# malaire/reed-solomon-16

Hardware: AMD Instinct MI355X
Metric: encode+decode GiB/s (device-resident, 1024B shards); % of HBM roofline (higher is better)
Workload: dtype u16; 1 GPU; 32768:32768 x 1024 B encode + 100%-loss decode per GPU (BASELINE configs[3]); original_count=32768, recovery_count=32768, parallelism=independent stripes x 1 (weak, no collective), column_slices=1, decode_issue=serial: rs16_decode_device after the encode

## Files before the change

include/rs16.h:

```cpp
#ifndef RS16_H
#define RS16_H

#include <stddef.h>
#include <stdint.h>

#ifdef __cplusplus
extern "C" {
#endif

typedef enum rs16_error_code {
    RS16_OK = 0,
    RS16_DIFFERENT_SHARD_SIZE = 1,
    RS16_DUPLICATE_ORIGINAL_SHARD_INDEX = 2,
    RS16_DUPLICATE_RECOVERY_SHARD_INDEX = 3,
    RS16_INVALID_ORIGINAL_SHARD_INDEX = 4,
    RS16_INVALID_RECOVERY_SHARD_INDEX = 5,
    RS16_INVALID_SHARD_SIZE = 6,
    RS16_NOT_ENOUGH_SHARDS = 7,
    RS16_TOO_FEW_ORIGINAL_SHARDS = 8,
    RS16_TOO_MANY_ORIGINAL_SHARDS = 9,
    RS16_UNSUPPORTED_SHARD_COUNT = 10,
    RS16_DEVICE_ERROR = 100,
    RS16_INVALID_ARGUMENT = 101
} rs16_error_code;
// ... 108 lines not shown
                        size_t original_received_count, size_t recovery_received_count, void* stream,
                        rs16_error* err);
int rs16_decode_device_prepared(rs16_engine* eng, size_t original_count, size_t recovery_count,
                                size_t shard_bytes, void* d_original, const void* d_recovery, void* stream,
                                rs16_error* err);

enum { RS16_UPDATE_MAX_SHARDS = 32 };
typedef struct rs16_update_plan rs16_update_plan;
rs16_update_plan* rs16_update_plan_new(rs16_engine* eng, int rate, size_t original_count, size_t recovery_count,
                                       const size_t* indices, size_t n, rs16_error* err);
void rs16_update_plan_free(rs16_update_plan* plan);
size_t rs16_update_plan_count(const rs16_update_plan* plan);
int rs16_update_plan_coefficients(rs16_update_plan* plan, uint16_t* out, rs16_error* err);
int rs16_update_device(rs16_update_plan* plan, size_t shard_bytes, const void* d_delta, void* d_recovery,
                       size_t recovery_pos, size_t recovery_n, void* stream, rs16_error* err);

int rs16_encode_host_batch(rs16_engine* eng, size_t original_count, size_t recovery_count, size_t shard_bytes,
                           size_t nstripes, const void* h_original, size_t original_stride, void* h_recovery,
                           size_t recovery_stride, rs16_error* err);
int rs16_decode_host_batch(rs16_engine* eng, size_t original_count, size_t recovery_count, size_t shard_bytes,
                           size_t nstripes, void* h_original, size_t original_stride,
                           const uint8_t* original_received, size_t original_received_stride,
                           const void* h_recovery, size_t recovery_stride, const uint8_t* recovery_received,
                           size_t recovery_received_stride, rs16_error* err);

int rs16_encode_host_multi(rs16_engine* const* engines, int n, size_t original_count, size_t recovery_count,
                           size_t shard_bytes, const void* h_original, void* h_recovery, rs16_error* err);
int rs16_decode_host_multi(rs16_engine* const* engines, int n, size_t original_count, size_t recovery_count,
                           size_t shard_bytes, void* h_original, const uint8_t* original_received,
                           const void* h_recovery, const uint8_t* recovery_received, rs16_error* err);

typedef struct rs16_comm rs16_comm;
int rs16_comm_unique_id(void* id128, rs16_error* err);
rs16_comm* rs16_comm_new(rs16_engine* eng, int nranks, int rank, const void* id128, rs16_error* err);
int rs16_comm_init_all(rs16_engine* const* engines, int n, rs16_comm** comms, rs16_error* err);
void rs16_comm_free(rs16_comm* comm);
int rs16_comm_rank(const rs16_comm* comm);
int rs16_comm_size(const rs16_comm* comm);
int rs16_column_slice(size_t shard_bytes, int nranks, int rank, size_t* offset, size_t* width);
int rs16_scatter_columns(rs16_comm* const* comms, int n, int root, size_t rows, size_t shard_bytes,
                         const void* const* d_full, void* const* d_slice, void* stream, rs16_error* err);
int rs16_gather_columns(rs16_comm* const* comms, int n, int root, size_t rows, size_t shard_bytes,
                        const void* const* d_slice, void* const* d_full, void* stream, rs16_error* err);
int rs16_scatter_columns_virtual(rs16_comm* comm, int vslices, size_t rows, size_t shard_bytes, const void* d_full,
                                 void* const* d_slices, void* stream, rs16_error* err);
int rs16_gather_columns_virtual(rs16_comm* comm, int vslices, size_t rows, size_t shard_bytes,
                                const void* const* d_slices, void* d_full, void* stream, rs16_error* err);

void* rs16_device_alloc(rs16_engine* eng, size_t bytes, rs16_error* err);
void rs16_device_free(rs16_engine* eng, void* d_ptr);
int rs16_memcpy_htod(rs16_engine* eng, void* d_dst, const void* src, size_t bytes, void* stream, rs16_error* err);
int rs16_memcpy_dtoh(rs16_engine* eng, void* dst, const void* d_src, size_t bytes, void* stream, rs16_error* err);
int rs16_memset_device(rs16_engine* eng, void* d_dst, int value, size_t bytes, void* stream, rs16_error* err);
int rs16_memcpy2d_htod(rs16_engine* eng, void* d_dst, size_t d_pitch, const void* src, size_t h_pitch, size_t width,
                       size_t rows, void* stream, rs16_error* err);
int rs16_memcpy2d_dtoh(rs16_engine* eng, void* dst, size_t h_pitch, const void* d_src, size_t d_pitch, size_t width,
                       size_t rows, void* stream, rs16_error* err);
void* rs16_stream_create(rs16_engine* eng, rs16_error* err);
void rs16_stream_destroy(rs16_engine* eng, void* stream);
void* rs16_host_alloc(rs16_engine* eng, size_t bytes, rs16_error* err);
void rs16_host_free(rs16_engine* eng, void* h_ptr);

int rs16_engine_set_profiling(rs16_engine* eng, int enable, rs16_error* err);
int rs16_engine_profile_read(rs16_engine* eng, int prog, double* total_ms, uint64_t* launches, rs16_error* err);
void rs16_engine_profile_reset(rs16_engine* eng);
int rs16_prog_count(void);
int rs16_engine_set_stamps(rs16_engine* eng, void* d_buf, int prog, rs16_error* err);
const char* rs16_prog_name(int prog);

enum {
    RS16_DIAG_FORCE_VOFF64 = 1,
    RS16_DIAG_EVAL_TWO_KERNEL = 2,
    RS16_DIAG_EVAL_FULL = 4,
    RS16_DIAG_NO_COLUMN = 8,
    RS16_DIAG_FORCE_COLUMN = 16,
    RS16_DIAG_TILE_LAST = 32,
    RS16_DIAG_NO_TILE_LAST = 64,
    RS16_DIAG_FD_LDS = 128,
    RS16_DIAG_COL_RADIX4 = 256,
    RS16_DIAG_NO_IDENTITY = 512,
    RS16_DIAG_NO_MID_DIRECT = 1024,
    RS16_DIAG_WIDE_TWIDDLES = 2048,
    RS16_DIAG_NO_LATE_ROWS = 4096,
    RS16_DIAG_NO_PAIRED_ROWS = 8192
};
int rs16_engine_set_diagnostics(rs16_engine* eng, int flags);
int rs16_set_diagnostics(int flags);

void rs16_host_mul(const void* in, void* out, size_t bytes, uint16_t log_m);
void rs16_host_mul_narrow(const void* in, void* out, size_t bytes, uint16_t log_m);
uint32_t rs16_host_twiddle(uint32_t index, uint32_t* log_m, uint32_t* table20);
int rs16_host_twiddle_narrow(uint32_t index);
uint64_t rs16_host_fast_div_check(uint32_t divisor, uint32_t n0, uint32_t count, uint32_t step);
typedef struct rs16_pass_consts {
    uint32_t voff32, full_lanes, nslab;
    uint32_t quads, threads, load_shb, store_shb, reg_bits, row_sets;
    uint64_t rs_in, rs_seg, rs_out;
    uint32_t late_rows;
} rs16_pass_consts;
int rs16_host_pass_consts(int prog, int T, uint32_t lo, uint64_t s_in, uint64_t s_out, uint64_t s_seg, uint64_t s_rest,
                          uint32_t qrow, uint32_t chunk, uint32_t row_base_in, uint32_t in_rows_mask, int diag,
                          rs16_pass_consts* out);
int rs16_host_pass_consts_many(int prog, int T, uint32_t lo, size_t n, const uint64_t* s_in, const uint64_t* s_out,
                               const uint64_t* s_seg, const uint64_t* s_rest, const uint32_t* qrow, uint32_t chunk,
                               uint32_t row_base_in, uint32_t in_rows_mask, int diag, rs16_pass_consts* out);
int rs16_host_pass_consts_rows(int prog, int T, uint32_t lo, uint64_t s_in, uint64_t s_out, uint64_t s_seg,
                               uint64_t s_rest, uint32_t qrow, uint32_t chunk, uint32_t row_base_in,
                               uint32_t in_rows_mask, uint32_t a_count, int diag, rs16_pass_consts* out);
int rs16_host_paired_rows(uint32_t chunk_rows, uint64_t S, uint64_t S_user, uint32_t a_count, uint32_t seg_chunk,
                          uint32_t row_base_in, int diag);
int rs16_host_update_consts(uint32_t rows, uint64_t shard_bytes, uint32_t n, uint32_t* quads_per_lane,
                            uint32_t* nslab, uint32_t* rows_per_wave, uint64_t* blocks);

const char* rs16_version(void);

#ifdef __cplusplus
}
#endif
#endif
```

reed-solomon-16_amd/csrc/rs16_api.cpp:

```cpp
#include <atomic>
#include <rccl/rccl.h>

#include <cstdio>

#include "rs16_api.hpp"
#include "rs16_pass_common.hpp"

using namespace rs16;

extern "C" size_t rs16_error_message(const rs16_error* e, char* buf, size_t len) {
    char tmp[256];
    unsigned long long a = e->v0, b = e->v1, c = e->v2;
    switch (e->code) {
    case RS16_OK: snprintf(tmp, sizeof tmp, "ok"); break;
    case RS16_DIFFERENT_SHARD_SIZE:
        snprintf(tmp, sizeof tmp, "different shard size: expected %llu bytes, got %llu bytes", a, b);
        break;
    case RS16_DUPLICATE_ORIGINAL_SHARD_INDEX: snprintf(tmp, sizeof tmp, "duplicate original shard index: %llu", a); break;
    case RS16_DUPLICATE_RECOVERY_SHARD_INDEX: snprintf(tmp, sizeof tmp, "duplicate recovery shard index: %llu", a); break;
    case RS16_INVALID_ORIGINAL_SHARD_INDEX:
        snprintf(tmp, sizeof tmp, "invalid original shard index: %llu >= original_count %llu", b, a);
        break;
    case RS16_INVALID_RECOVERY_SHARD_INDEX:
        snprintf(tmp, sizeof tmp, "invalid recovery shard index: %llu >= recovery_count %llu", b, a);
        break;
    case RS16_INVALID_SHARD_SIZE:
        snprintf(tmp, sizeof tmp, "invalid shard size: %llu bytes (must non-zero and multiple of 64)", a);
        break;
    case RS16_NOT_ENOUGH_SHARDS:
        snprintf(tmp, sizeof tmp, "not enough shards: %llu original + %llu recovery < %llu original_count", b, c, a);
        break;
    case RS16_TOO_FEW_ORIGINAL_SHARDS:
        snprintf(tmp, sizeof tmp, "too few original shards: got %llu shards while original_count is %llu", b, a);
        break;
    case RS16_TOO_MANY_ORIGINAL_SHARDS:
        snprintf(tmp, sizeof tmp, "too many original shards: got more than original_count (%llu) shards", a);
        break;
    case RS16_UNSUPPORTED_SHARD_COUNT:
        snprintf(tmp, sizeof tmp, "unsupported shard count: %llu original shards with %llu recovery shards", a, b);
        break;
    case RS16_DEVICE_ERROR:
        if (a >= 1000)
            snprintf(tmp, sizeof tmp, "device error: RCCL: %s", ncclGetErrorString((ncclResult_t)(a - 1000)));
        else
            snprintf(tmp, sizeof tmp, "device error: %s", hipGetErrorString((hipError_t)a));
        break;
    case RS16_INVALID_ARGUMENT: snprintf(tmp, sizeof tmp, "invalid argument"); break;
    default: snprintf(tmp, sizeof tmp, "unknown error %d", e->code); break;
    }
    size_t n = strlen(tmp);
    if (buf && len) {
        size_t c2 = std::min(n, len - 1);
        memcpy(buf, tmp, c2);
        buf[c2] = 0;
    }
    return n;
}

template <class Mul> static void host_mul(const void* in, void* out, size_t bytes, uint16_t log_m, Mul mul) {
    const uint32_t* t = &host_tables().mul_tab[(size_t)log_m * TAB_DWORDS];
    const uint8_t* src = (const uint8_t*)in;
    uint8_t* dst = (uint8_t*)out;
    for (size_t q = 0; q < bytes / 8; q++) {
        const size_t off = (q >> 3) * 64 + (q & 7) * 4;
        uint32_t yl, yh, ol = 0, oh = 0;
        memcpy(&yl, src + off, 4);
        memcpy(&yh, src + off + 32, 4);
        mul(ol, oh, yl, yh, t);
        memcpy(dst + off, &ol, 4);
        memcpy(dst + off + 32, &oh, 4);
    }
}
extern "C" void rs16_host_mul(const void* in, void* out, size_t bytes, uint16_t log_m) {
    host_mul(in, out, bytes, log_m, mul_xor);
}
extern "C" void rs16_host_mul_narrow(const void* in, void* out, size_t bytes, uint16_t log_m) {
    host_mul(in, out, bytes, log_m, mul_xor_narrow);
}
extern "C" uint32_t rs16_host_twiddle(uint32_t index, uint32_t* log_m, uint32_t* table20) {
    const HostTables& t = host_tables();
    if (index >= GF_MODULUS) return ~0u;
    if (log_m) *log_m = t.skew[index];
    if (table20) memcpy(table20, &t.skew_tab[(size_t)index * TAB_DWORDS], 20 * sizeof(uint32_t));
    return t.skew[index] == GF_MODULUS ? 0u : t.exp[t.skew[index]];
}
extern "C" int rs16_host_twiddle_narrow(uint32_t index) { return twiddle_narrow(index) ? 1 : 0; }
extern "C" uint64_t rs16_host_fast_div_check(uint32_t divisor, uint32_t n0, uint32_t count, uint32_t step) {
    const FastDiv f = fast_div_of(divisor);
    uint64_t bad = 0;
    for (uint64_t i = 0, n = n0; i < count && n < ((uint64_t)1 << 32); i++, n += step)
        bad += fast_div((uint32_t)n, f.mul, f.one) != (uint32_t)n / divisor;
    return bad;
}

static int host_pass_consts(int prog, int T, uint32_t lo, size_t n, const uint64_t* s_in, const uint64_t* s_out,
                            const uint64_t* s_seg, const uint64_t* s_rest, const uint32_t* qrow, uint32_t chunk,
                            uint32_t row_base_in, uint32_t in_rows_mask, uint32_t a_count, int diag,
                            rs16_pass_consts* out) {
    if (prog < 0 || prog >= NUM_PROGS || T < 0 || T > 8 || !out) return 0;
    const PassKernel& k = pass_kernel_of(prog, T);
    if (!k.fn) return 0;
    PassArgs a{};
    a.lo = lo, a.chunk = chunk, a.row_base_in = row_base_in, a.in_rows_mask = in_rows_mask;
    a.diag = (uint32_t)diag;
    a.a_count = a_count;
    for (size_t i = 0; i < n; i++) {
        a.S_in = s_in[i], a.S_out = s_out[i], a.S_seg = s_seg[i], a.S_rest = s_rest[i], a.qrow = qrow[i];
        const PassConsts c = pass_launch_consts(k, T, a);
        rs16_pass_consts& o = out[i];
        o.voff32 = c.voff32, o.full_lanes = c.full_lanes, o.nslab = c.nslab;
        o.quads = (uint32_t)k.quads, o.threads = (uint32_t)k.threads;
        o.load_shb = (uint32_t)k.load_shb, o.store_shb = (uint32_t)k.store_shb;
        o.reg_bits = (uint32_t)k.reg_bits, o.row_sets = k.quads >= 64 ? 1u : 64u / (uint32_t)k.quads;
        o.rs_in = c.rs_in, o.rs_seg = c.rs_seg, o.rs_out = c.rs_out;
        o.late_rows = c.late_rows;
    }
    return 1;
}
extern "C" int rs16_host_pass_consts_many(int prog, int T, uint32_t lo, size_t n, const uint64_t* s_in,
                                          const uint64_t* s_out, const uint64_t* s_seg, const uint64_t* s_rest,
                                          const uint32_t* qrow, uint32_t chunk, uint32_t row_base_in,
                                          uint32_t in_rows_mask, int diag, rs16_pass_consts* out) {
    return host_pass_consts(prog, T, lo, n, s_in, s_out, s_seg, s_rest, qrow, chunk, row_base_in, in_rows_mask, 0, diag,
                            out);
}
extern "C" int rs16_host_pass_consts_rows(int prog, int T, uint32_t lo, uint64_t s_in, uint64_t s_out, uint64_t s_seg,
                                          uint64_t s_rest, uint32_t qrow, uint32_t chunk, uint32_t row_base_in,
                                          uint32_t in_rows_mask, uint32_t a_count, int diag, rs16_pass_consts* out) {
    return host_pass_consts(prog, T, lo, 1, &s_in, &s_out, &s_seg, &s_rest, &qrow, chunk, row_base_in, in_rows_mask,
                            a_count, diag, out);
}
extern "C" int rs16_host_pass_consts(int prog, int T, uint32_t lo, uint64_t s_in, uint64_t s_out, uint64_t s_seg,
                                     uint64_t s_rest, uint32_t qrow, uint32_t chunk, uint32_t row_base_in,
                                     uint32_t in_rows_mask, int diag, rs16_pass_consts* out) {
    return rs16_host_pass_consts_many(prog, T, lo, 1, &s_in, &s_out, &s_seg, &s_rest, &qrow, chunk, row_base_in,
                                      in_rows_mask, diag, out);
}
extern "C" int rs16_host_paired_rows(uint32_t chunk_rows, uint64_t S, uint64_t S_user, uint32_t a_count,
                                     uint32_t seg_chunk, uint32_t row_base_in, int diag) {
    return paired_rows_sequence(chunk_rows, S, S_user, a_count, seg_chunk, row_base_in, diag) ? 1 : 0;
}
extern "C" int rs16_host_update_consts(uint32_t rows, uint64_t shard_bytes, uint32_t n, uint32_t* quads_per_lane,
                                       uint32_t* nslab, uint32_t* rows_per_wave, uint64_t* blocks) {
    if (shard_bytes == 0 || (shard_bytes & 63) != 0 || shard_bytes / 8 > 0xFFFFFFFFu) return 0;
    UpdateArgs a{};
    a.S = shard_bytes, a.qrow = (uint32_t)(shard_bytes / 8), a.rows = rows;
    uint64_t nb;
    if (!update_launch_consts(a, n, &nb)) return 0;
    if (quads_per_lane) *quads_per_lane = a.quads_per_lane;
    if (nslab) *nslab = a.nslab;
    if (rows_per_wave) *rows_per_wave = a.rows_per_wave;
    if (blocks) *blocks = nb;
    return 1;
}

extern "C" int rs16_engine_set_profiling(rs16_engine* e, int enable, rs16_error* err) {
    if (int rc = e->activate(err)) return rc;
    if (int rc = e->prof_collect(err)) return rc;
    e->profiling = enable != 0;
    return set_error(err, RS16_OK);
}
extern "C" int rs16_engine_profile_read(rs16_engine* e, int prog, double* total_ms, uint64_t* launches,
                                        rs16_error* err) {
    if (prog < 0 || prog >= NUM_PROF) return set_error(err, RS16_INVALID_ARGUMENT);
    if (int rc = e->activate(err)) return rc;
    if (int rc = e->prof_collect(err)) return rc;
    if (total_ms) *total_ms = e->prof_ms[prog];
    if (launches) *launches = e->prof_n[prog];
    return set_error(err, RS16_OK);
}
extern "C" void rs16_engine_profile_reset(rs16_engine* e) {
    rs16_error err;
    (void)e->activate(&err);
    (void)e->prof_collect(&err);
    for (int i = 0; i < NUM_PROF; i++) e->prof_ms[i] = 0, e->prof_n[i] = 0;
}
extern "C" int rs16_engine_set_stamps(rs16_engine* e, void* d_buf, int prog, rs16_error* err) {
    if (prog < -1 || prog >= NUM_PROF) return set_error(err, RS16_INVALID_ARGUMENT);
    e->stamp_buf = d_buf;
    e->stamp_prof = prog;
    return set_error(err, RS16_OK);
}
extern "C" int rs16_engine_set_slices(rs16_engine* e, int n, rs16_error* err) {
    if (n < 1 || n > rs16_engine::MAX_SLICES) return set_error(err, RS16_INVALID_ARGUMENT);
    e->slices = n;
    return set_error(err, RS16_OK);
}
extern "C" int rs16_decode_check(rs16_engine* e, void* stream, rs16_error* err) {
    if (!e->last_dec_valid && !e->last_dec_flags_only) return set_error(err, RS16_OK);
    if (int rc = e->activate(err)) return rc;
    RS16_HIP(hipStreamSynchronize(e->pick(stream)));
    const DecodeGeom& g = e->last_dec;
    uint64_t a = 0, b = 0;
    if (e->last_dec_flags_only) {
        std::vector<uint8_t> f(2 * (size_t)GF_ORDER);
        RS16_HIP(hipMemcpy(f.data(), e->ws_flags.p, f.size(), hipMemcpyDeviceToHost));
        for (uint32_t i = 0; i < g.a_count; i++) a += f[i] != 0;
        for (uint32_t i = 0; i < g.b_count; i++) b += f[GF_ORDER + i] != 0;
    } else {
        const size_t chunks = ((size_t)g.n + 63) / 64;
        std::vector<uint32_t> c(2 * chunks);
        RS16_HIP(hipMemcpy(c.data(), e->ev_main.rcount.p, c.size() * 4, hipMemcpyDeviceToHost));
        for (size_t i = 0; i < chunks; i++) a += c[2 * i], b += c[2 * i + 1];
    }
    const auto want = DecodeSides::by_segment<uint64_t>(g.high, g.a_recv, g.b_recv);
    const auto got = DecodeSides::by_segment<uint64_t>(g.high, a, b);
    if (got != want) return set_error(err, RS16_INVALID_ARGUMENT, got.first, got.second);
    return set_error(err, RS16_OK);
}
static constexpr int DIAG_ALL = DIAG_FORCE_VOFF64 | DIAG_EVAL_TWO_KERNEL | DIAG_EVAL_FULL | DIAG_NO_COLUMN |
                                DIAG_FORCE_COLUMN | DIAG_TILE_LAST | DIAG_NO_TILE_LAST | DIAG_FD_LDS |
                                DIAG_COL_RADIX4 | DIAG_NO_IDENTITY | DIAG_NO_MID_DIRECT | DIAG_WIDE_TWIDDLES |
                                DIAG_NO_LATE_ROWS | DIAG_NO_PAIRED_ROWS;
extern "C" int rs16_engine_set_diagnostics(rs16_engine* e, int flags) {
    const int old = e->diag;
    e->diag = flags & DIAG_ALL;
    return old;
}
static std::atomic<int> g_default_diag{0};
extern "C" int rs16_set_diagnostics(int flags) { return g_default_diag.exchange(flags & DIAG_ALL); }
extern "C" int rs16_prog_count(void) { return NUM_PROF; }
extern "C" const char* rs16_prog_name(int prog) {
    static const char* names[] = {"GEN_FFT",   "GEN_IFFT",   "ENC_FIRST",     "ENC_MID",
                                  "ENC_LAST",  "ENC_SINGLE", "DEC_FIRST",     "DEC_MID",
                                  "DEC_LAST",  "DEC_SINGLE", "DEC_HALF_LAST", "DEC_HALF_SINGLE",
                                  "DEC_HALF_FIRST", "DEC_HALF_MID", "EVAL_POLY", "COL_ENC", "COL_DEC",
                                  "DEC_MID_DIRECT", "DEC_TILE_LAST"};
    static_assert(sizeof names / sizeof names[0] == NUM_PROF, "profiling names");
    return (prog >= 0 && prog < NUM_PROF) ? names[prog] : "?";
}

extern "C" const char* rs16_version(void) { return "rs16-mi355x 0.1 gfx950 (v_perm GF(2^16) engine)"; }

static bool high_supports(size_t k, size_t m) {
    return k > 0 && m > 0 && k < GF_ORDER && m < GF_ORDER && next_pow2(m) + k <= GF_ORDER;
}
static bool low_supports(size_t k, size_t m) {
    return k > 0 && m > 0 && k < GF_ORDER && m < GF_ORDER && next_pow2(k) + m <= GF_ORDER;
}

extern "C" int rs16_use_high_rate(size_t k, size_t m, rs16_error* err) {
    if (k > GF_ORDER || m > GF_ORDER) return set_error(err, RS16_UNSUPPORTED_SHARD_COUNT, k, m), -1;
    const size_t kp = next_pow2(k), mp = next_pow2(m);
    const size_t smaller = std::min(kp, mp), larger = std::max(k, m);
    if (k == 0 || m == 0 || smaller + larger > GF_ORDER) return set_error(err, RS16_UNSUPPORTED_SHARD_COUNT, k, m), -1;
    set_error(err, RS16_OK);
    if (kp < mp) return 0;
    if (kp > mp) return 1;
    return k <= m ? 1 : 0;
}

extern "C" int rs16_supports(int rate, size_t k, size_t m) {
    if (rate == RS16_RATE_HIGH) return high_supports(k, m);
    if (rate == RS16_RATE_LOW) return low_supports(k, m);
    return rs16_use_high_rate(k, m, nullptr) >= 0;
}

extern "C" int rs16_validate(int rate, size_t k, size_t m, size_t S, rs16_error* err) {
    if (!rs16_supports(rate, k, m)) return set_error(err, RS16_UNSUPPORTED_SHARD_COUNT, k, m);
    if (S == 0 || (S & 63) != 0 || (uint64_t)S >> 32) return set_error(err, RS16_INVALID_SHARD_SIZE, S);
    return set_error(err, RS16_OK);
}

extern "C" size_t rs16_encoder_work_count(int high, size_t k, size_t m) {
    const size_t chunk = high ? next_pow2(m) : next_pow2(k);
    const size_t n = high ? k : m;
    return (n + chunk - 1) / chunk * chunk;
}
extern "C" size_t rs16_decoder_work_count(int high, size_t k, size_t m) {
    return decode_geom(high != 0, k, m).n;
}

int rs16::resolve_rate(int rate, size_t k, size_t m, size_t S, bool* high, rs16_error* err) {
    if (rate == RS16_RATE_DEFAULT) {
        int h = rs16_use_high_rate(k, m, err);
        if (h < 0) return err ? err->code : RS16_UNSUPPORTED_SHARD_COUNT;
        *high = h == 1;
    } else if (rate == RS16_RATE_HIGH || rate == RS16_RATE_LOW) {
        *high = rate == RS16_RATE_HIGH;
    } else {
        return set_error(err, RS16_INVALID_ARGUMENT);
    }
    return rs16_validate(*high ? RS16_RATE_HIGH : RS16_RATE_LOW, k, m, S, err);
}
int rs16::check_received(size_t k, size_t orig_recv, size_t rec_recv, rs16_error* err) {
    if (orig_recv + rec_recv < k) return set_error(err, RS16_NOT_ENOUGH_SHARDS, k, orig_recv, rec_recv);
    return RS16_OK;
}

extern "C" rs16_engine* rs16_engine_new(int device, rs16_error* err) { return rs16_engine_new_ex(device, 0, err); }

extern "C" rs16_engine* rs16_engine_new_ex(int device, int flags, rs16_error* err) {
    if (flags & ~RS16_ENGINE_OWN_QUEUE) return set_error(err, RS16_INVALID_ARGUMENT), nullptr;
    int ndev = 0;
    hipError_t he = hipGetDeviceCount(&ndev);
    if (he != hipSuccess) return hip_fail(err, he), nullptr;
    if (device < 0 || device >= ndev) return set_error(err, RS16_INVALID_ARGUMENT), nullptr;
    rs16_engine* e = new (std::nothrow) rs16_engine();
    if (!e) return set_error(err, RS16_INVALID_ARGUMENT), nullptr;
    e->device = device;
    e->diag = g_default_diag.load();
    const HostTables& t = host_tables();
    auto fail = [&](hipError_t x) {
        hip_fail(err, x);
        rs16_engine_free(e);
        return (rs16_engine*)nullptr;
    };
    if ((he = hipSetDevice(device)) != hipSuccess) return fail(he);
    if (flags & RS16_ENGINE_OWN_QUEUE) {
        int cus = 0;
        if ((he = hipDeviceGetAttribute(&cus, hipDeviceAttributeMultiprocessorCount, device)) != hipSuccess) return fail(he);
        std::vector<uint32_t> mask(((size_t)cus + 31) / 32, 0xFFFFFFFFu);
        if (cus % 32) mask.back() = (1u << (cus % 32)) - 1;
        if ((he = hipExtStreamCreateWithCUMask(&e->stream, (uint32_t)mask.size(), mask.data())) != hipSuccess)
            return fail(he);
    } else if ((he = hipStreamCreateWithFlags(&e->stream, hipStreamNonBlocking)) != hipSuccess) {
        return fail(he);
    }
    e->flags = flags;
    if ((he = hipMalloc(&e->d_skew_tab, (size_t)GF_ORDER * TAB_DWORDS * 4)) != hipSuccess) return fail(he);
    if ((he = hipMalloc(&e->d_mul_tab, t.mul_tab.size() * 4)) != hipSuccess) return fail(he);
    if ((he = hipMalloc(&e->d_log_walsh, GF_ORDER * 2)) != hipSuccess) return fail(he);
    if ((he = hipMalloc(&e->d_zero_sink, RS16_ZERO_BYTES)) != hipSuccess) return fail(he);
    if ((he = hipMemset(e->d_zero_sink, 0, RS16_ZERO_BYTES)) != hipSuccess) return fail(he);
    if ((he = hipMemcpy(e->d_skew_tab, t.skew_tab.data(), t.skew_tab.size() * 4, hipMemcpyHostToDevice)) != hipSuccess) return fail(he);
    if ((he = hipMemcpy(e->d_mul_tab, t.mul_tab.data(), t.mul_tab.size() * 4, hipMemcpyHostToDevice)) != hipSuccess) return fail(he);
    if ((he = hipMemcpy(e->d_log_walsh, t.log_walsh.data(), GF_ORDER * 2, hipMemcpyHostToDevice)) != hipSuccess) return fail(he);
    set_error(err, RS16_OK);
    return e;
}

extern "C" void rs16_engine_free(rs16_engine* e) {
    if (!e) return;
    (void)hipSetDevice(e->device);
    if (e->stream) (void)hipStreamSynchronize(e->stream);
    for (int j = 0; j < rs16_engine::MAX_SLICES; j++)
        if (e->sl_own[j]) (void)hipStreamSynchronize(e->sl_own[j]);
    for (auto& sl : e->hslot)
        if (sl.s) (void)hipStreamSynchronize(sl.s);
    if (e->last == rs16_engine::LAST_CALLER && e->order_ev) (void)hipEventSynchronize(e->order_ev);
    for (rs16_encoder* c : e->encoders) detach(c);
    for (rs16_decoder* c : e->decoders) detach(c);
    for (rs16_update_plan* c : e->update_plans) detach(c);
    e->ws_z.release();
    e->ws_u.release();
    e->ws_fd.release();
    for (auto& b : e->mid_tab) b.release();
    e->ev_main.release();
    for (auto& l : e->ev_lane) l.release();
    e->ws_flags.release();
    e->hp_flags.release();
    for (auto& sl : e->hslot) {
        if (sl.s) (void)hipStreamSynchronize(sl.s), (void)hipStreamDestroy(sl.s);
        sl.orig.release(), sl.rec.release(), sl.z.release(), sl.u.release();
    }
    e->hflags.release();
    if (e->hev) (void)hipEventDestroy(e->hev);
    if (e->prep_ev) (void)hipEventDestroy(e->prep_ev);
    for (auto& ev : e->hp_ev)
        if (ev) (void)hipEventDestroy(ev);
    if (e->hp_off) (void)hipEventDestroy(e->hp_off);
    if (e->order_ev) (void)hipEventDestroy(e->order_ev);
    for (int j = 0; j < rs16_engine::MAX_SLICES; j++) {
        if (e->sl_own[j]) (void)hipStreamDestroy(e->sl_own[j]);
        if (e->sl_join[j]) (void)hipEventDestroy(e->sl_join[j]);
    }
    if (e->sl_fork) (void)hipEventDestroy(e->sl_fork);
    if (e->d_skew_tab) (void)hipFree(e->d_skew_tab);
    if (e->d_mul_tab) (void)hipFree(e->d_mul_tab);
    if (e->d_col_img) (void)hipFree(e->d_col_img);
    if (e->d_col_v) (void)hipFree(e->d_col_v);
    if (e->d_log_walsh) (void)hipFree(e->d_log_walsh);
    if (e->d_zero_sink) (void)hipFree(e->d_zero_sink);
    if (e->stream) (void)hipStreamDestroy(e->stream);
    delete e;
}

extern "C" int rs16_engine_device(const rs16_engine* e) { return e->device; }
extern "C" void* rs16_engine_stream(const rs16_engine* e) { return (void*)e->stream; }
extern "C" int rs16_engine_synchronize(rs16_engine* e, void* stream, rs16_error* err) {
    if (int rc = e->activate(err)) return rc;
    RS16_HIP(hipStreamSynchronize(e->pick(stream)));
    return set_error(err, RS16_OK);
}

static bool is_pow2(size_t x) { return x && !(x & (x - 1)); }

static int check_transform(size_t shard_count, size_t S, size_t pos, size_t size, size_t trunc, size_t skew_delta,
                           rs16_error* err) {
    if (S == 0 || (S & 63) || !is_pow2(size) || size > GF_ORDER || trunc > size || pos + size > shard_count)
        return set_error(err, RS16_INVALID_ARGUMENT);
    if (size >= 2 && size - 2 + skew_delta >= GF_MODULUS) return set_error(err, RS16_INVALID_ARGUMENT);
    return RS16_OK;
}

extern "C" int rs16_engine_fft(rs16_engine* e, void* data, size_t shard_count, size_t S, size_t pos, size_t size,
                               size_t trunc, size_t skew_delta, void* stream, rs16_error* err) {
    if (int rc = check_transform(shard_count, S, pos, size, trunc, skew_delta, err)) return rc;
    if (!shard_aligned(data)) return set_error(err, RS16_INVALID_ARGUMENT);
    if (int rc = e->activate(err)) return rc;
    if (int rc = e->fft((uint8_t*)data, S, pos, size, skew_delta, e->pick(stream), err)) return rc;
    return set_error(err, RS16_OK);
}
extern "C" int rs16_engine_fft_skew_end(rs16_engine* e, void* data, size_t shard_count, size_t S, size_t pos,
                                        size_t size, size_t trunc, void* stream, rs16_error* err) {
    return rs16_engine_fft(e, data, shard_count, S, pos, size, trunc, pos + size, stream, err);
}
extern "C" int rs16_engine_ifft(rs16_engine* e, void* data, size_t shard_count, size_t S, size_t pos, size_t size,
                                size_t trunc, size_t skew_delta, void* stream, rs16_error* err) {
    if (int rc = check_transform(shard_count, S, pos, size, trunc, skew_delta, err)) return rc;
    if (!shard_aligned(data)) return set_error(err, RS16_INVALID_ARGUMENT);
    if (int rc = e->activate(err)) return rc;
    if (int rc = e->ifft((uint8_t*)data, S, pos, size, skew_delta, e->pick(stream), err)) return rc;
    return set_error(err, RS16_OK);
}
extern "C" int rs16_engine_ifft_skew_end(rs16_engine* e, void* data, size_t shard_count, size_t S, size_t pos,
                                         size_t size, size_t trunc, void* stream, rs16_error* err) {
    return rs16_engine_ifft(e, data, shard_count, S, pos, size, trunc, pos + size, stream, err);
}
extern "C" int rs16_engine_fwht(rs16_engine* e, uint16_t* d, size_t trunc, void* stream, rs16_error* err) {
    if (trunc > GF_ORDER) return set_error(err, RS16_INVALID_ARGUMENT);
    if (int rc = e->activate(err)) return rc;
    if (int rc = e->order(e->pick(stream), err)) return rc;
    if (int rc = e->guard_eval(e->pick(stream), false, err)) return rc;
    RS16_HIP(e->evset->work32.reserve(GF_ORDER * 4));
    RS16_HIP(launch_fwht_u16(d, (uint32_t*)e->evset->work32.p, e->pick(stream)));
    if (int rc = e->scratch_done(e->pick(stream), err)) return rc;
    return set_error(err, RS16_OK);
}
extern "C" int rs16_engine_eval_poly(rs16_engine* e, uint16_t* d, size_t trunc, void* stream, rs16_error* err) {
    if (trunc > GF_ORDER) return set_error(err, RS16_INVALID_ARGUMENT);
    if (int rc = e->activate(err)) return rc;
    if (int rc = e->order(e->pick(stream), err)) return rc;
    if (int rc = e->guard_eval(e->pick(stream), false, err)) return rc;
    RS16_HIP(e->evset->work32.reserve(GF_ORDER * 4));
    RS16_HIP(launch_eval_poly_u16(d, (uint32_t*)e->evset->work32.p, e->d_log_walsh, e->pick(stream)));
    if (int rc = e->scratch_done(e->pick(stream), err)) return rc;
    return set_error(err, RS16_OK);
}
extern "C" int rs16_engine_mul(rs16_engine* e, void* x, size_t bytes, uint16_t log_m, void* stream, rs16_error* err) {
    if ((bytes & 63) || !shard_aligned(x)) return set_error(err, RS16_INVALID_ARGUMENT);
    if (int rc = e->activate(err)) return rc;
    RS16_HIP(launch_mul((uint8_t*)x, bytes, log_m, e->d_mul_tab, e->pick(stream)));
    return set_error(err, RS16_OK);
}
extern "C" int rs16_engine_xor(rs16_engine* e, void* x, const void* y, size_t bytes, void* stream, rs16_error* err) {
    if ((bytes & 63) || !shard_aligned(x) || !shard_aligned(y)) return set_error(err, RS16_INVALID_ARGUMENT);
    if (int rc = e->activate(err)) return rc;
    RS16_HIP(launch_xor((uint8_t*)x, (const uint8_t*)y, bytes, e->pick(stream)));
    return set_error(err, RS16_OK);
}
// ... 88 lines not shown
```

reed-solomon-16_amd/csrc/rs16_engine.cpp:

```cpp
#include <cstdlib>
#include "rs16_engine.hpp"

#include <algorithm>
#include <cstring>

namespace rs16 {

hipError_t DevBuf::reserve(size_t bytes) {
    if (bytes <= cap) return hipSuccess;
    if (p) (void)hipFree(p);
    p = nullptr;
    cap = 0;
    hipError_t e = hipMalloc(&p, bytes);
    if (e == hipSuccess) cap = bytes;
    return e;
}
void DevBuf::release() {
    if (p) (void)hipFree(p);
    p = nullptr;
    cap = 0;
}

hipError_t HostBuf::reserve(size_t bytes) {
    if (bytes <= cap) return hipSuccess;
// ... 265 lines not shown
}

int rs16_engine::fft(uint8_t* data, size_t S, size_t pos, size_t size, size_t skew_delta, hipStream_t s,
                     rs16_error* err) {
    const int L = ilog2(size);
    if (L == 0) return RS16_OK;
    PassArgs a = base_args(this, S);
    a.in = a.out = data + pos * S;
    a.skew_fft = (uint32_t)skew_delta;
    if (L <= 8) {
        RS16_PASS(GEN_FFT, L, a, 1, s);
        return RS16_OK;
    }
    const int lo = L / 2, hi = L - lo;
    a.lo = lo;
    RS16_PASS(GEN_FFT, hi, a, 1u << lo, s);
    a.lo = 0;
    RS16_PASS(GEN_FFT, lo, a, 1u << hi, s);
    return RS16_OK;
}

int rs16_engine::ifft(uint8_t* data, size_t S, size_t pos, size_t size, size_t skew_delta, hipStream_t s,
                      rs16_error* err) {
    const int L = ilog2(size);
    if (L == 0) return RS16_OK;
    PassArgs a = base_args(this, S);
    a.in = a.out = data + pos * S;
    a.skew_ifft = (uint32_t)skew_delta;
    if (L <= 8) {
        RS16_PASS(GEN_IFFT, L, a, 1, s);
        return RS16_OK;
    }
    const int lo = L / 2, hi = L - lo;
    a.lo = 0;
    RS16_PASS(GEN_IFFT, lo, a, 1u << hi, s);
    a.lo = lo;
    RS16_PASS(GEN_IFFT, hi, a, 1u << lo, s);
    return RS16_OK;
}

int rs16_engine::encode_high_fused(size_t k, size_t m, size_t S, size_t S_user, const uint8_t* d_orig, uint8_t* d_rec, uint8_t* Z,
                                   hipStream_t s, rs16_error* err, size_t nst, size_t bs_orig, size_t bs_rec) {
    const size_t chunk = next_pow2(m);
    const int L = ilog2(chunk);
    PassArgs a = base_args(this, S);
    a.seg_a = d_orig;
    a.S_seg = S_user;
    a.a_count = (uint32_t)k;
    a.skew_ifft = (uint32_t)chunk;
    a.skew_fft = 0;
    a.out_rows = (uint32_t)m;
    const uint32_t ns = (uint32_t)nst;
    auto batch = [&](uint32_t tiles, size_t bs_in, size_t bs_out, size_t bs_seg) {
        a.stripe_tiles = ns > 1 ? tiles : 0;
        a.bs_in = bs_in;
        a.bs_out = bs_out;
        a.bs_seg = bs_seg;
        return tiles * ns;
    };
    if (col_ok(L, S, nst)) {
        ColArgs c = col_args();
        c.in = d_orig;
        c.out = d_rec;
        c.S_in = c.S_out = S_user;
        c.qrow = (uint32_t)(S / 8);
        c.nstripes = ns;
        c.bs_in = bs_orig;
        c.bs_out = bs_rec;
        c.in_rows = (uint32_t)k;
        c.out_rows = (uint32_t)m;
        c.skew_ifft = (uint32_t)chunk;
        c.skew_fft = 0;
        return col(c, L, COL_ENC, s, err);
    }
    if (L <= 8) {
        a.out = d_rec;
        a.S_out = S_user;
        RS16_PASS(ENC_SINGLE, L, a, batch(1, 0, bs_rec, bs_orig), s);
        return RS16_OK;
    }
    const int lo = L / 2, hi = L - lo;
    const size_t zs = chunk * S;
    const bool paired = paired_rows_sequence((uint32_t)chunk, S, S_user, a.a_count, a.chunk, a.row_base_in, diag);
    a.out = Z;
    a.lo = 0;
    a.paired = paired ? paired_sides_of(ENC_FIRST) : 0;
    RS16_PASS(ENC_FIRST, lo, a, batch(1u << hi, 0, zs, bs_orig), s);
    a.in = Z;
    a.lo = lo;
    a.paired = paired ? paired_sides_of(ENC_MID) : 0;
    RS16_PASS(ENC_MID, hi, a, batch(1u << lo, zs, zs, 0), s);
    a.in = Z;
    a.out = d_rec;
    a.S_out = S_user;
    a.lo = 0;
    a.paired = paired ? paired_sides_of(ENC_LAST) : 0;
    const uint32_t tiles = (uint32_t)((m + ((size_t)1 << lo) - 1) >> lo);
    RS16_PASS(ENC_LAST, lo, a, batch(tiles, zs, bs_rec, 0), s);
    return RS16_OK;
}

int rs16_engine::decode_fused(const DecodeGeom& g, size_t S, size_t S_user, const uint8_t* seg_a, const uint8_t* flags_a,
                              const uint8_t* seg_b, const uint8_t* flags_b, uint8_t* rest, uint8_t* Z, uint8_t* U,
                              hipStream_t s, rs16_error* err) {
    if (int rc = decode_eval(g, flags_a, flags_b, s, err, S)) return rc;
    return decode_passes(g, S, S_user, seg_a, flags_a, seg_b, flags_b, rest, Z, U, (uint32_t*)evset->rcount.p, s, err);
}

int rs16_engine::guard_eval(hipStream_t s, bool consume, rs16_error* err) {
    if (!prep_pending) return RS16_OK;
    RS16_HIP(hipStreamWaitEvent(s, prep_ev, 0));
    prep_pending = false;
    if (!consume) prep.valid = false;
    return RS16_OK;
}

int rs16_engine::decode_eval(const DecodeGeom& g, const uint8_t* flags_a, const uint8_t* flags_b, hipStream_t s,
                             rs16_error* err, size_t S, size_t nstripes, uint32_t vary, size_t bs_fa, size_t bs_fb) {
    if (evset == &ev_main && !preparing)
        if (int rc = guard_eval(s, false, err)) return rc;
    if (!preparing) prep.valid = false;
    const size_t nv = vary > 1 ? vary : 1;
    RS16_HIP(evset->work32.reserve(nv * VARY_WORK * 4));
    RS16_HIP(evset->elog.reserve(nv * VARY_WORK * 4));
    RS16_HIP(evset->zflag.reserve(nv * VARY_ZFLAGS));
    RS16_HIP(evset->rbits.reserve(nv * VARY_RBITS * 4));
    RS16_HIP(evset->lost.reserve(nv * VARY_LOST * 4));
    RS16_HIP(evset->rcount.reserve(GF_ORDER / 64 * 8));
    var_ns = vary > 1 ? vary : 0;
    var_bs_fa = vary > 1 ? bs_fa : 0;
    var_bs_fb = vary > 1 ? bs_fb : 0;
    ErasureSpec es{};
    es.flags_a = flags_a;
    es.flags_b = flags_b;
    es.a_count = g.a_count;
    es.chunk = g.chunk;
    es.b_count = g.b_count;
    es.pad_fill = g.high ? 1 : 0;
    es.tail_fill = g.high ? 0 : 1;
    const int L = ilog2(g.n);
    es.rbits = (uint32_t*)evset->rbits.p;
    es.zflags = L > 8 ? (uint8_t*)evset->zflag.p : nullptr;
    es.n = g.n;
    es.zlo = (uint32_t)(L / 2);
    const bool prune = !half_decode(g) && L > 8;
    es.lostpart = prune ? (uint32_t*)evset->lost.p : nullptr;
    es.lostrange = prune ? (uint32_t*)evset->lost.p + 512 : nullptr;
    es.orig_b = g.high ? 1 : 0;
    es.rcount = (uint32_t*)evset->rcount.p;
    es.diag = (uint32_t)diag;
    last_dec = g;
    last_dec_valid = true;
    if (var_ns) {
        es.nstripes = var_ns;
        es.bs_fa = var_bs_fa;
        es.bs_fb = var_bs_fb;
        es.bs_work = es.bs_elog = VARY_WORK;
        es.bs_rbits = VARY_RBITS;
        es.bs_zflags = VARY_ZFLAGS;
        es.bs_lost = VARY_LOST;
        es.rcount = nullptr;
        last_dec_valid = false;
    }
    e_ident = identity_logs(g, vary);
    if (e_ident) {
        eval_in_col = elog_fused = false;
        return RS16_OK;
    }
    eval_in_col = S && (half_decode(g) ? g.high && col_ok(ilog2(g.n) - 1, S, nstripes)
                                       : col_ok(ilog2(g.n), S, nstripes, true));
    if (eval_in_col) return RS16_OK;
    es.stamps = stamp_prof == PROF_EVAL_POLY ? (uint64_t*)stamp_buf : nullptr;
    hipEvent_t pev;
    if (int rc = prof_begin(s, &pev, err)) return rc;
    const bool small = g.high && g.n <= 2048 && !(diag & DIAG_EVAL_FULL);
    elog_fused = !(half_decode(g) && ilog2(g.n) - 1 <= 8);
    if (small) {
        RS16_HIP(launch_eval_poly_small(es, (uint32_t)g.n, (uint32_t*)evset->work32.p, (uint32_t*)evset->elog.p, d_log_walsh,
                                        s, !elog_fused));
// ... 11 lines not shown

bool rs16_engine::identity_logs(const DecodeGeom& g, uint32_t vary) const {
    if ((diag & DIAG_NO_IDENTITY) || vary > 1 || !half_decode(g) || ilog2(g.n) - 1 < 11) return false;
    if (g.a_count != g.chunk || g.b_count != g.chunk) return false;
    return g.high ? g.a_recv == g.a_count : g.b_recv == g.b_count;
}

int rs16_engine::mid_tables(int L, const uint32_t** out, rs16_error* err) {
    DevBuf& b = mid_tab[L];
    if (!b.p) {
        const HostTables& t = host_tables();
        const std::vector<uint32_t> ent = mid_matrix_entries(t, L);
        std::vector<uint32_t> tabs(ent.size() * 20);
        for (size_t i = 0; i < ent.size(); i++)
            std::copy_n(&t.mul_tab[(size_t)ent[i] * TAB_DWORDS], 20, &tabs[i * 20]);
        hipError_t he = b.reserve(tabs.size() * 4);
        if (he == hipSuccess) he = hipMemcpy(b.p, tabs.data(), tabs.size() * 4, hipMemcpyHostToDevice);
        if (he != hipSuccess) {
            b.release();
            return hip_fail(err, he);
        }
    }
    *out = (const uint32_t*)b.p;
    return RS16_OK;
}

int rs16_engine::decode_passes(const DecodeGeom& g, size_t S, size_t S_user, const uint8_t* seg_a, const uint8_t* flags_a,
                               const uint8_t* seg_b, const uint8_t* flags_b, uint8_t* rest, uint8_t* Z, uint8_t* U,
                               uint32_t* rcount, hipStream_t s, rs16_error* err, size_t nst, size_t bs_a, size_t bs_b,
                               size_t bs_rest) {
    PassArgs a = base_args(this, S);
    a.S_seg = a.S_rest = S_user;
    a.seg_a = seg_a;
    a.seg_b = seg_b;
    a.flags_a = flags_a;
    a.flags_b = flags_b;
    a.a_count = g.a_count;
    a.chunk = g.chunk;
    a.b_count = g.b_count;
    a.elog = (const uint32_t*)evset->elog.p;
    a.ework = elog_fused ? (const uint32_t*)evset->work32.p : nullptr;
    a.rest = rest;
    a.rest_seg_b = g.high ? 1 : 0;
    a.rbits = (const uint32_t*)evset->rbits.p;
    a.skew_ifft = a.skew_fft = 0;
    if (var_ns) {
        a.bs_fa = var_bs_fa;
        a.bs_fb = var_bs_fb;
        a.bs_elog = VARY_WORK;
        a.bs_rbits = VARY_RBITS;
        a.bs_zflags = VARY_ZFLAGS;
        a.bs_lost = VARY_LOST;
        rcount = nullptr;
    }
    const uint32_t ns = (uint32_t)nst;
    const size_t zs = (size_t)g.n * S;
    a.bs_seg = bs_a;
    a.bs_seg_b = bs_b;
    a.bs_rest = bs_rest;
    auto batch = [&](uint32_t tiles, size_t bs_in, size_t bs_in2, size_t bs_out) {
        a.stripe_tiles = ns > 1 ? tiles : 0;
        a.bs_in = bs_in;
        a.bs_in2 = bs_in2;
        a.bs_out = bs_out;
        return tiles * ns;
    };
    const int L = ilog2(g.n);
    if (half_decode(g)) {
        const uint32_t half = g.n / 2, src = g.high ? 0 : half, dst = g.high ? half : 0;
        const uint32_t orig = g.high ? g.b_count : g.a_count;
        a.row_base_in = a.skew_ifft = src;
        a.row_base_out = a.skew_fft = dst;
        const int Lh = L - 1;
        if (e_ident) {
            const int lo = Lh / 2, hi = Lh - lo;
            a.seg_a = g.high ? seg_a : seg_b;
            a.bs_seg = g.high ? bs_a : bs_b;
            a.a_count = half;
            a.rcount = rcount;
            a.cnt_flags = g.high ? flags_a : flags_b;
            a.cnt_base = src;
            a.cnt_seg = g.high ? 0 : 1;
            const bool paired = paired_rows_sequence(half, S, S_user, a.a_count, a.chunk, a.row_base_in, diag);
            a.lo = 0;
            a.out = Z;
            a.paired = paired ? paired_sides_of(ENC_FIRST) : 0;
            RS16_PASS_AS(PROF_DEC_HALF_FIRST, ENC_FIRST, lo, a, batch(1u << hi, 0, 0, zs), s);
            a.rcount = nullptr;
            a.lo = lo;
            a.in = Z;
            a.paired = paired ? paired_sides_of(ENC_MID) : 0;
            RS16_PASS_AS(PROF_DEC_HALF_MID, ENC_MID, hi, a, batch(1u << lo, zs, 0, zs), s);
            a.lo = 0;
            a.out = rest;
            a.S_out = S_user;
            a.out_rows = orig;
            a.paired = paired ? paired_sides_of(ENC_LAST) : 0;
            a.rcount = rcount;
            a.cnt_flags = g.high ? flags_b : flags_a;
            a.cnt_base = dst;
            a.cnt_seg = g.high ? 1 : 0;
            RS16_PASS_AS(DEC_HALF_LAST, ENC_LAST, lo, a, batch((orig + (1u << lo) - 1) >> lo, zs, 0, bs_rest), s);
            return RS16_OK;
        }
        const bool col_eval = eval_in_col && g.high;
        if (!col_eval && Lh <= 8) {
            a.ework = nullptr;
            RS16_PASS(DEC_HALF_SINGLE, Lh, a, batch(1, 0, 0, 0), s);
            return RS16_OK;
        }
        if (col_eval || col_ok(Lh, S, ns)) {
            ColArgs c = col_args();
            c.in = g.high ? seg_a : seg_b;
            c.flags = g.high ? flags_a : flags_b;
            c.in_rows = g.high ? g.a_count : g.b_count;
            c.out = rest;
            c.S_in = c.S_out = S_user;
            c.qrow = (uint32_t)(S / 8);
            c.nstripes = ns;
            c.bs_in = g.high ? bs_a : bs_b;
            c.bs_out = bs_rest;
            c.out_rows = orig;
            c.base_in = c.skew_ifft = src;
            c.base_out = c.skew_fft = dst;
            c.chunk = g.chunk;
            c.e_pad = 1;
            c.bs_flags = g.high ? var_bs_fa : var_bs_fb;
            c.bs_flags_o = var_bs_fb;
            c.bs_elog = var_ns ? VARY_WORK : 0;
            if (col_eval) {
                c.flags_o = flags_b;
                c.o_rows = g.b_count;
                c.vtab = nullptr;
                c.rcount = rcount;
                return col(c, Lh, COL_DEC_EVAL, s, err);
            }
            c.elog = (const uint32_t*)evset->work32.p;
            return col(c, Lh, COL_DEC_EWORK, s, err);
        }
        const int lo = Lh / 2, hi = Lh - lo;
        a.paired = 0;
        a.lo = 0;
        a.out = Z;
        RS16_PASS_AS(PROF_DEC_HALF_FIRST, DEC_FIRST, lo, a, batch(1u << hi, 0, 0, zs), s);
        a.lo = lo;
        a.in = Z;
        RS16_PASS_AS(PROF_DEC_HALF_MID, ENC_MID, hi, a, batch(1u << lo, zs, 0, zs), s);
        a.lo = 0;
        a.out = nullptr;
        RS16_PASS(DEC_HALF_LAST, lo, a, batch((orig + (1u << lo) - 1) >> lo, zs, 0, 0), s);
        return RS16_OK;
    }
    if (eval_in_col) {
        ColArgs c = col_args();
        c.in = seg_a;
        c.flags = flags_a;
        c.in_rows = g.a_count;
        c.in_b = seg_b;
        c.bs_in_b = bs_b;
        c.flags_o = flags_b;
        c.o_rows = g.b_count;
        c.chunk = g.chunk;
        c.rev_a = g.high ? 0 : 1;
        c.e_pad = g.high ? 1 : 0;
        c.e_tail = g.high ? 0 : 1;
        c.e_k = g.high ? 0 : host_tables().col_k[L];
        c.out = rest;
        c.S_in = c.S_out = S_user;
        c.qrow = (uint32_t)(S / 8);
        c.nstripes = ns;
        c.bs_in = bs_a;
        c.bs_out = bs_rest;
        c.out_rows = g.high ? g.b_count : g.a_count;
        c.rcount = rcount;
        c.bs_flags = var_bs_fa;
        c.bs_flags_o = var_bs_fb;
        return col(c, L, COL_DEC_GEN, s, err);
    }
    if (L <= 8) {
        RS16_PASS(DEC_SINGLE, L, a, batch(1, 0, 0, 0), s);
// ... 206 lines not shown
```

reed-solomon-16_amd/csrc/rs16_engine.hpp:

```cpp
#pragma once
#include <cstddef>
#include <cstdint>
#include <vector>

#include "../../include/rs16.h"
#include "rs16_internal.hpp"

namespace rs16 {

struct DevBuf {
    void* p = nullptr;
    size_t cap = 0;
    hipError_t reserve(size_t bytes);
    void release();
};
struct HostBuf {
    void* p = nullptr;
    size_t cap = 0;
    hipError_t reserve(size_t bytes);
    void release();
};
struct Pending {
    hipEvent_t ev = nullptr;
    bool busy = false;
    hipError_t record(hipStream_t s);
    hipError_t wait();
    void release();
};

int set_error(rs16_error* err, int code, uint64_t v0 = 0, uint64_t v1 = 0, uint64_t v2 = 0);
int hip_fail(rs16_error* err, hipError_t e);
#define RS16_HIP(call)                                 \
    do {                                               \
        hipError_t _e = (call);                        \
        if (_e != hipSuccess) return hip_fail(err, _e); \
    } while (0)
#define RS16_PASS(...)                                       \
    do {                                                     \
        if (int _rc = this->pass(__VA_ARGS__, err)) return _rc; \
    } while (0)
#define RS16_PASS_AS(PROF, ...)                                     \
    do {                                                            \
        if (int _rc = this->pass(__VA_ARGS__, err, PROF)) return _rc; \
    } while (0)

size_t next_pow2(size_t x);
inline int ilog2(size_t x) { int l = 0; while (((size_t)1 << l) < x) l++; return l; }

struct DecodeGeom {
    bool high;
    uint32_t a_count, chunk, b_count, n;
    size_t a_recv = 1, b_recv = 1;
};
DecodeGeom decode_geom(bool high, size_t k, size_t m);

}

struct rs16_encoder;
struct rs16_decoder;
struct rs16_update_plan;

struct rs16_engine {
    int device = 0;
    int flags = 0;
    hipStream_t stream = nullptr;
    int diag = 0;
    uint32_t* d_skew_tab = nullptr;
    uint32_t* d_mul_tab = nullptr;
    uint32_t* d_col_img = nullptr;
    uint32_t* d_col_v = nullptr;
    uint16_t* d_log_walsh = nullptr;
    uint8_t* d_zero_sink = nullptr;
    rs16::DevBuf ws_z, ws_u, ws_fd, ws_flags;
    rs16::DevBuf mid_tab[17];
    struct EvalBufs {
        rs16::DevBuf work32, elog;
        rs16::DevBuf zflag;
        rs16::DevBuf rbits;
        rs16::DevBuf lost;
        rs16::DevBuf rcount;
        void release() { work32.release(), elog.release(), zflag.release(), rbits.release(), lost.release(), rcount.release(); }
    };
    EvalBufs ev_main, ev_lane[2];
    EvalBufs* evset = &ev_main;
    struct Prepared {
        bool valid = false, nothing = false;
        size_t k = 0, m = 0, S = 0;
        rs16::DecodeGeom g{};
        const uint8_t* fl_a = nullptr;
        const uint8_t* fl_b = nullptr;
        int nslices = 1;
    } prep;
    hipEvent_t prep_ev = nullptr;
    bool prep_pending = false;
    bool preparing = false;
    int guard_eval(hipStream_t s, bool consume, rs16_error* err);
    rs16::DecodeGeom last_dec{};
    bool last_dec_valid = false;
    bool last_dec_flags_only = false;
    void forget_decode() { last_dec_valid = last_dec_flags_only = false; }
    struct HostSlot {
        hipStream_t s = nullptr;
        rs16::DevBuf orig, rec, z, u;
        rs16::DevBuf rcount;
    };
    HostSlot hslot[2];
    static constexpr int MAX_SLICES = 4;
    int slices = 1;
    hipStream_t sl_stream[MAX_SLICES] = {};
    hipStream_t sl_own[MAX_SLICES] = {};
    hipEvent_t sl_fork = nullptr, sl_join[MAX_SLICES] = {};
    int slice_count(size_t S) const;
    int fork(hipStream_t s, int n, rs16_error* err);
    int join(hipStream_t s, int n, rs16_error* err);
    rs16::DevBuf hflags;
    hipEvent_t hev = nullptr;
    hipEvent_t hp_ev[2] = {};
    hipEvent_t hp_off = nullptr;
    rs16::HostBuf hp_flags;
    int host_pipe_events(rs16_error* err);
    int host_slots(rs16_error* err);

    hipStream_t pick(void* s) const { return s ? (hipStream_t)s : stream; }
    int activate(rs16_error* err);

    enum { LAST_NONE, LAST_ENGINE, LAST_CALLER } last = LAST_NONE;
    hipEvent_t order_ev = nullptr;
    int order(hipStream_t s, rs16_error* err);
    int scratch_done(hipStream_t s, rs16_error* err);

    std::vector<rs16_encoder*> encoders;
    std::vector<rs16_decoder*> decoders;
    std::vector<rs16_update_plan*> update_plans;

    int pass(int prog, int T, const rs16::PassArgs& a, uint32_t tiles, hipStream_t s, rs16_error* err,
             int prof = -1);
    int prof_begin(hipStream_t s, hipEvent_t* ev, rs16_error* err);
    int prof_end(int id, hipStream_t s, hipEvent_t ev, rs16_error* err);
    template <class F> int profiled(int prof, hipStream_t s, rs16_error* err, F launch);
    bool profiling = false;
    void* stamp_buf = nullptr;
    int stamp_prof = -1;
    bool elog_fused = false;
    bool eval_in_col = false;
    bool e_ident = false;
    struct ProfRec {
        int id;
        hipEvent_t a, b;
    };
    std::vector<ProfRec> prof_pending;
// ... 44 lines not shown
```

reed-solomon-16_amd/csrc/rs16_gf.hpp:

```cpp
#pragma once
#include <stdint.h>

#if defined(__HIPCC__) || defined(__HIP__)
#include <hip/hip_runtime.h>
#define RS16_HD __host__ __device__ __forceinline__
#else
#define RS16_HD inline
#endif

namespace rs16 {

constexpr uint32_t GF_ORDER = 65536;
constexpr uint32_t GF_MODULUS = 65535;
constexpr uint32_t ZERO_ENTRY = 65536;
constexpr uint32_t TAB_ENTRIES = 65537;
constexpr uint32_t TAB_DWORDS = 32;

RS16_HD uint32_t perm_sw(uint32_t hi, uint32_t lo, uint32_t sel) {
    uint64_t pool = ((uint64_t)hi << 32) | lo;
    uint32_t r = 0;
    for (int i = 0; i < 4; i++) {
        uint32_t s = (sel >> (8 * i)) & 0xFF;
        r |= (uint32_t)((pool >> (8 * s)) & 0xFF) << (8 * i);
    }
    return r;
}

#if defined(__HIP_DEVICE_COMPILE__)
__device__ __forceinline__ uint32_t perm(uint32_t hi, uint32_t lo, uint32_t sel) {
    return __builtin_amdgcn_perm(hi, lo, sel);
}
__device__ __forceinline__ uint32_t xor3(uint32_t a, uint32_t b, uint32_t c) {
    return __builtin_amdgcn_bitop3_b32(a, b, c, 0x96);
}
#else
inline uint32_t perm(uint32_t hi, uint32_t lo, uint32_t sel) { return perm_sw(hi, lo, sel); }
inline uint32_t xor3(uint32_t a, uint32_t b, uint32_t c) { return a ^ b ^ c; }
#endif

struct MulSel {
    uint32_t s0, s1, s2, s3, s4, s5;
};
RS16_HD MulSel mul_selectors(uint32_t yL, uint32_t yH) {
#if defined(__HIP_DEVICE_COMPILE__)
    const uint64_t y = ((uint64_t)yH << 32) | yL;
    uint64_t a, b;
    asm("v_lshrrev_b64 %0, 3, %1" : "=v"(a) : "v"(y));
    asm("v_lshrrev_b64 %0, 6, %1" : "=v"(b) : "v"(y));
    const uint32_t s0 = yL & 0x07070707u;
    const uint32_t s1 = (uint32_t)a & 0x07070707u;
    const uint32_t s2 = (uint32_t)b & 0x03030303u;
    const uint32_t s3 = yH & 0x07070707u;
    const uint32_t s4 = (uint32_t)(a >> 32) & 0x07070707u;
    const uint32_t s5 = (uint32_t)(b >> 32) & 0x03030303u;
#else
    const uint32_t s0 = yL & 0x07070707u;
    const uint32_t a = yL >> 3;
    const uint32_t s1 = a & 0x07070707u;
    const uint32_t s2 = (a >> 3) & 0x03030303u;
    const uint32_t s3 = yH & 0x07070707u;
    const uint32_t b = yH >> 3;
    const uint32_t s4 = b & 0x07070707u;
    const uint32_t s5 = (b >> 3) & 0x03030303u;
#endif
    return MulSel{s0, s1, s2, s3, s4, s5};
}
template <bool NARROW>
RS16_HD void mul_xor_sel(uint32_t& xL, uint32_t& xH, const MulSel& y, const uint32_t* t) {
    const uint32_t s0 = y.s0, s1 = y.s1, s2 = y.s2, s3 = y.s3, s4 = y.s4, s5 = y.s5;
    if constexpr (NARROW) {
        const uint32_t l0 = perm(t[1], t[0], s0);
        const uint32_t l1 = perm(t[5], t[4], s1);
        const uint32_t l3 = perm(t[9], t[8], s3), h3 = perm(t[11], t[10], s3);
        const uint32_t l4 = perm(t[13], t[12], s4), h4 = perm(t[15], t[14], s4);
        const uint32_t l2 = perm(t[16], t[16], s2);
        const uint32_t l5 = perm(t[18], t[18], s5), h5 = perm(t[19], t[19], s5);
        xL = xor3(xor3(xL, l0, l1), xor3(l2, l3, l4), l5);
        xH = xor3(xH, h3, h4) ^ h5;
    } else {
        const uint32_t l0 = perm(t[1], t[0], s0), h0 = perm(t[3], t[2], s0);
        const uint32_t l1 = perm(t[5], t[4], s1), h1 = perm(t[7], t[6], s1);
        const uint32_t l3 = perm(t[9], t[8], s3), h3 = perm(t[11], t[10], s3);
        const uint32_t l4 = perm(t[13], t[12], s4), h4 = perm(t[15], t[14], s4);
        const uint32_t l2 = perm(t[16], t[16], s2), h2 = perm(t[17], t[17], s2);
        const uint32_t l5 = perm(t[18], t[18], s5), h5 = perm(t[19], t[19], s5);
        xL = xor3(xor3(xL, l0, l1), xor3(l2, l3, l4), l5);
        xH = xor3(xor3(xH, h0, h1), xor3(h2, h3, h4), h5);
    }
}
template <bool NARROW>
RS16_HD void mul_xor_t(uint32_t& xL, uint32_t& xH, uint32_t yL, uint32_t yH, const uint32_t* t) {
    mul_xor_sel<NARROW>(xL, xH, mul_selectors(yL, yH), t);
}
RS16_HD void mul_xor(uint32_t& xL, uint32_t& xH, uint32_t yL, uint32_t yH, const uint32_t* t) {
    mul_xor_t<false>(xL, xH, yL, yH, t);
}
RS16_HD void mul_xor_narrow(uint32_t& xL, uint32_t& xH, uint32_t yL, uint32_t yH, const uint32_t* t) {
    mul_xor_t<true>(xL, xH, yL, yH, t);
}

RS16_HD uint32_t add_mod(uint32_t x, uint32_t y) {
    uint32_t s = x + y;
    return (s + (s >> 16)) & 0xFFFFu;
}
RS16_HD uint32_t sub_mod(uint32_t x, uint32_t y) {
    uint32_t d = x - y;
    return (d + (d >> 16)) & 0xFFFFu;
}

}
```

reed-solomon-16_amd/csrc/rs16_internal.hpp:

```cpp
#pragma once
#include <hip/hip_runtime.h>
#include <stddef.h>
#include <stdint.h>

#include <vector>

#include "rs16_gf.hpp"

namespace rs16 {

struct HostTables {
    std::vector<uint16_t> exp, log, skew, log_walsh;
    std::vector<uint32_t> skew_entry;
    std::vector<uint32_t> mul_tab;
    std::vector<uint32_t> skew_tab;
    std::vector<uint32_t> col_img;
    std::vector<uint32_t> col_v;
    std::vector<uint32_t> col_k;
};
std::vector<uint32_t> mid_matrix_entries(const HostTables& t, int L);

constexpr uint32_t COL_LMIN = 6, COL_LMAX = 10;
constexpr uint32_t COL_LGEN = 11;
constexpr uint32_t COL_LCHUNK = 8;
constexpr uint32_t col_img_count(uint32_t L) {
    return L == COL_LGEN ? 1u : (L >= COL_LCHUNK ? (1u << (16 - L)) : 2u);
}
constexpr size_t col_img_offset(uint32_t L, uint32_t d) {
    size_t off = 0;
    for (uint32_t l = COL_LMIN; l < L; l++) off += (size_t)col_img_count(l) * ((1u << l) - 1) * 20;
    return off + (size_t)d * ((1u << L) - 1) * 20;
}
constexpr size_t COL_IMG_DWORDS = col_img_offset(COL_LGEN + 1, 0);
constexpr size_t col_v_offset(uint32_t n) { return n - (1u << COL_LMIN); }
constexpr size_t COL_V_DWORDS = col_v_offset(4u << COL_LMAX);
const HostTables& host_tables();

RS16_HD bool twiddle_narrow(uint32_t i) {
    const uint32_t x = i + 1;
    return x < ((x & (0u - x)) << 8);
}
inline int first_narrow_layer(uint32_t lo, int T, uint32_t skew, uint32_t bh_max) {
    int k = T;
    for (int kb = T - 1; kb >= 0; kb--) {
        const uint64_t d = (uint64_t)1 << (lo + kb);
        const uint64_t xmax = (((uint64_t)bh_max + 1) << (lo + T)) - d + skew;
        const uint64_t low = (d + skew) & (2 * d - 1);
        const uint64_t bit = low ? (low & (0 - low)) : 2 * d;
        if (xmax >= (bit << 8)) break;
        k = kb;
    }
    return k;
}

enum Prog : int {
    GEN_FFT = 0,
    GEN_IFFT,
    ENC_FIRST,
    ENC_MID,
    ENC_LAST,
    ENC_SINGLE,
    DEC_FIRST,
    DEC_MID,
    DEC_LAST,
    DEC_SINGLE,
    DEC_HALF_LAST,
    DEC_HALF_SINGLE,
    NUM_PROGS
};
enum ProfId : int {
    PROF_DEC_HALF_FIRST = NUM_PROGS,
    PROF_DEC_HALF_MID,
    PROF_EVAL_POLY,
    PROF_COL_ENC,
    PROF_COL_DEC,
    PROF_DEC_MID_DIRECT,
    PROF_DEC_TILE_LAST,
    NUM_PROF
};

struct PassArgs {
    uint8_t* out;
    const uint8_t* in;
    const uint8_t* in2;
    const uint8_t* seg_a;
    const uint8_t* seg_b;
    const uint8_t* flags_a;
    const uint8_t* flags_b;
    uint8_t* rest;
    const uint32_t* elog;
    const uint32_t* skew_tab;
    const uint32_t* mul_tab;
    uint64_t S_in, S_out, S_seg, S_rest;
    uint32_t qrow;
    uint32_t nslab;
    uint32_t ntiles;
    uint32_t lo;
    uint32_t a_count, chunk, b_count;
// ... 16 lines not shown
    uint32_t in_rows_mask;
    uint64_t bs_fa, bs_fb;
    uint32_t bs_elog, bs_rbits, bs_zflags, bs_lost;
    uint32_t diag;
    uint32_t* rcount;
    const uint8_t* cnt_flags;
    uint32_t cnt_base, cnt_seg;
    uint32_t mid_direct;
    uint32_t tl_max;
    uint64_t rs_in, rs_seg, rs_out;
    uint32_t full_lanes;
    uint32_t nslab_one, stripe_one;
    uint32_t paired;
    uint64_t nslab_mul, stripe_mul;
};

struct FastDiv {
    uint64_t mul;
    uint32_t one;
};
inline FastDiv fast_div_of(uint32_t d) {
    if (d <= 1) return {0, ~0u};
    return {~(uint64_t)0 / d + 1, 0};
}
RS16_HD uint32_t fast_div(uint32_t n, uint64_t mul, uint32_t one) {
    const uint64_t lo = ((uint64_t)n * (uint32_t)mul) >> 32;
    return (uint32_t)(((uint64_t)n * (uint32_t)(mul >> 32) + lo) >> 32) + (n & one);
}

struct ColArgs {
    const uint8_t* img_ifft;
    const uint8_t* img_fft;
    const uint8_t* flags_o;
    uint32_t o_rows;
    const uint32_t* vtab;
    uint32_t* rcount;
    uint32_t chunk;
    uint32_t e_pad, e_tail, e_k;
    uint32_t rev_a;
    const uint8_t* in_b;
    uint64_t bs_in_b;
    const uint8_t* in;
    const uint8_t* flags;
    uint8_t* out;
    const uint32_t* elog;
    const uint32_t* skew_tab;
    const uint32_t* mul_tab;
    const uint8_t* zero;
    uint64_t S_in, S_out;
    uint32_t qrow;
    uint32_t nstripes;
    uint32_t in_rows, out_rows;
    uint32_t skew_ifft, skew_fft;
    uint32_t base_in, base_out;
    uint64_t bs_in, bs_out;
    uint64_t bs_flags, bs_flags_o;
    uint32_t bs_elog;
    uint32_t nch;
    uint64_t* stamps;
    uint32_t diag;
};
int col_rows_ok(uint32_t L);
enum ColMode : int { COL_ENC = 0, COL_DEC_EWORK, COL_DEC_EVAL, COL_DEC_GEN, COL_ENC_IFFT, COL_ENC_FFTX };
constexpr uint32_t COL_MAX_CHUNKS = 64;
hipError_t launch_col(const ColArgs& a, uint32_t L, int mode, hipStream_t s);
constexpr uint32_t COLM_L = 7, COLM_MAX_CHUNKS = 16;
hipError_t launch_col_multi(const ColArgs& a, bool high, hipStream_t s);

enum DiagFlags : int {
    DIAG_FORCE_VOFF64 = 1,
    DIAG_EVAL_TWO_KERNEL = 2,
    DIAG_EVAL_FULL = 4,
    DIAG_NO_COLUMN = 8,
    DIAG_FORCE_COLUMN = 16,
    DIAG_TILE_LAST = 32,
    DIAG_NO_TILE_LAST = 64,
    DIAG_FD_LDS = 128,
    DIAG_COL_RADIX4 = 256,
    DIAG_NO_IDENTITY = 512,
    DIAG_NO_MID_DIRECT = 1024,
    DIAG_WIDE_TWIDDLES = 2048,
    DIAG_NO_LATE_ROWS = 4096,
    DIAG_NO_PAIRED_ROWS = 8192,
};

constexpr size_t RS16_ZERO_BYTES = 65536;

hipError_t launch_pass(int prog, int T, const PassArgs& a, uint32_t num_tiles, hipStream_t s);
bool paired_rows_sequence(uint32_t chunk_rows, uint64_t S, uint64_t S_user, uint32_t a_count, uint32_t seg_chunk,
                          uint32_t row_base_in, int diag);
enum PairedSides : uint32_t { PAIRED_IN = 1, PAIRED_OUT = 2 };
inline uint32_t paired_sides_of(int prog) {
    return prog == ENC_FIRST ? PAIRED_OUT : prog == ENC_MID ? PAIRED_IN | PAIRED_OUT : prog == ENC_LAST ? PAIRED_IN : 0u;
}
hipError_t launch_tile_last(const PassArgs& a, uint32_t num_tiles, hipStream_t s);
constexpr uint32_t MID_DIRECT_MAX = 4;
constexpr uint32_t TILE_LAST_MAX = 16;
hipError_t launch_mid_direct(const PassArgs& a, const uint32_t* mtab, uint32_t hi, uint32_t ns, hipStream_t s);

hipError_t launch_mul(uint8_t* x, size_t bytes, uint32_t entry, const uint32_t* mul_tab, hipStream_t s);
hipError_t launch_xor(uint8_t* x, const uint8_t* y, size_t bytes, hipStream_t s);
hipError_t launch_xor_chunks(uint8_t* w, size_t chunk_bytes, uint32_t nch, hipStream_t s);
hipError_t launch_copy_chunks(uint8_t* w, size_t chunk_bytes, uint32_t nch, hipStream_t s);
hipError_t launch_formal_derivative(uint8_t* out, const uint8_t* in, size_t shard_count, size_t S, hipStream_t s);

constexpr uint32_t UPDATE_MAX_SHARDS = 32;
struct UpdateArgs {
    uint8_t* rec;
    const uint8_t* delta;
    const uint32_t* idx;
    const uint32_t* mul_tab;
    uint64_t S;
    uint32_t qrow;
    uint32_t row0, rows;
    uint32_t quads_per_lane, nslab, rows_per_wave;
};
bool update_launch_consts(UpdateArgs& a, uint32_t n, uint64_t* blocks);
hipError_t launch_update(UpdateArgs a, uint32_t n, hipStream_t s);

struct ErasureSpec {
    const uint8_t* flags_a;
    const uint8_t* flags_b;
    uint32_t a_count, chunk, b_count;
    uint32_t pad_fill;
    uint32_t tail_fill;
    uint32_t* rbits;
    uint8_t* zflags;
    uint32_t n, zlo;
    uint32_t* lostpart;
    uint32_t* lostrange;
    uint32_t orig_b;
    uint32_t* rcount;
    uint64_t* stamps;
    uint32_t nstripes;
    uint64_t bs_fa, bs_fb;
    uint32_t bs_work, bs_elog, bs_rbits, bs_zflags, bs_lost;
    uint32_t diag;
};
hipError_t launch_eval_poly_from_flags(const ErasureSpec& e, uint32_t* work, uint32_t* out_elog,
                                       const uint16_t* log_walsh, hipStream_t s, bool last_lo);
hipError_t launch_eval_poly_small(const ErasureSpec& e, uint32_t n, uint32_t* work, uint32_t* out_elog,
                                  const uint16_t* log_walsh, hipStream_t s, bool last_lo);
hipError_t launch_eval_poly_u16(uint16_t* data, uint32_t* work, const uint16_t* log_walsh, hipStream_t s);
hipError_t launch_fwht_u16(uint16_t* data, uint32_t* work, hipStream_t s);

}
```

reed-solomon-16_amd/csrc/rs16_pass.hpp:

```cpp
#pragma once
#include <type_traits>

#include "rs16_pass_common.hpp"
#include "rs16_fwht.hpp"
#include "rs16_diag.hpp"

namespace rs16 {

enum LoadMode { LD_PLAIN = 0, LD_GATHER_ENC, LD_GATHER_DEC, LD_DEC_LAST };
enum StoreMode { ST_PLAIN = 0, ST_RECOVERY, ST_RESTORE };

template <int P> struct ProgTraits;
#define RS16_PROG(P, LD, I, F, FF, ST)          \
    template <> struct ProgTraits<P> {         \
        static constexpr int LOAD = LD;        \
        static constexpr bool IFFT = I;        \
        static constexpr bool FD = F;          \
        static constexpr bool FFT = FF;        \
        static constexpr int STORE = ST;       \
        static constexpr bool ST_NT = !(I && FF);                                           \
    };
RS16_PROG(GEN_FFT, LD_PLAIN, false, false, true, ST_PLAIN)
RS16_PROG(GEN_IFFT, LD_PLAIN, true, false, false, ST_PLAIN)
RS16_PROG(ENC_FIRST, LD_GATHER_ENC, true, false, false, ST_PLAIN)
// ... 366 lines not shown
        return row_lost_original(a, r) ? GF_MODULUS - (el ? el[k] : a.elog[r]) : ZERO_ENTRY;
    }
};

struct NoFin {
    template <class X> __device__ __forceinline__ void operator()(const X&, const X&, int) const {}
};
struct NoPre {
    template <class X> __device__ __forceinline__ void operator()(X&, X&, int) const {}
};

template <int T, bool LB, int KB0, int KB1, bool FFT> struct LayerSeq {
    static constexpr int SH = LB ? Geo<T>::SHB : 0;
    static constexpr int NR = Geo<T>::NR;
    static constexpr bool DF = FFT && !LB && KB0 == 0 && KB1 == Geo<T>::R && NR >= 8;
    static constexpr int df_at(int g) {
        int skb[16] = {}, sgi[16] = {};
        int sp = 0, n = 0;
        skb[sp] = KB1 - 1, sgi[sp] = 0, sp++;
        while (sp > 0) {
            sp--;
            const int kb = skb[sp], gi = sgi[sp];
            if (n++ == g) return kb * 16 + gi;
            if (kb > 0) {
                skb[sp] = kb - 1, sgi[sp] = 2 * gi + 1, sp++;
                skb[sp] = kb - 1, sgi[sp] = 2 * gi, sp++;
            }
        }
        return 0;
    }
    static constexpr int kb_of(int s) { return FFT ? KB1 - 1 - s : KB0 + s; }
    static constexpr int groups_of(int s) { return NR >> (kb_of(s) - SH + 1); }
    static constexpr int total() {
        int n = 0;
        for (int s = 0; s < KB1 - KB0; s++) n += groups_of(s);
        return n;
    }
    static constexpr int step_of(int g) {
        if (DF) return KB1 - 1 - df_at(g) / 16;
        int s = 0;
        while (g >= groups_of(s)) g -= groups_of(s), s++;
        return s;
    }
    static constexpr int index_of(int g) {
        if (DF) return df_at(g) % 16;
        int s = 0;
        while (g >= groups_of(s)) g -= groups_of(s), s++;
        return g;
    }
};

template <int T, bool LB, int KB0, int KB1, bool FFT, int G, bool IN_TAB2>
__device__ __forceinline__ const uint4* group_table(const Thr& c, const uint4* tab1, const uint4* tab2) {
    using S = LayerSeq<T, LB, KB0, KB1, FFT>;
    constexpr int s = S::step_of(G), gi = S::index_of(G);
    constexpr int kb = S::kb_of(s);
    constexpr int off = (1 << T) - (1 << (T - kb));
    const uint32_t j = LB ? (uint32_t)gi : (c.s << (Geo<T>::R - 1 - kb)) + gi;
    const uint32_t t = off + j;
    constexpr uint32_t base2 = T > 4 ? Geo<T>::TSPLIT : 0;
    return IN_TAB2 ? tab2 + (t - base2) * 5 : tab1 + t * 5;
}

template <int NR> __device__ __forceinline__ void pin_rows(uint32_t (&L)[NR], uint32_t (&H)[NR]) {
    if constexpr (NR >= 4) {
#pragma unroll
        for (int i = 0; i < NR; i += 4)
            asm volatile("" : "+v"(L[i]), "+v"(L[i + 1]), "+v"(L[i + 2]), "+v"(L[i + 3]), "+v"(H[i]), "+v"(H[i + 1]),
                         "+v"(H[i + 2]), "+v"(H[i + 3]));
    } else {
#pragma unroll
        for (int i = 0; i < NR; i++) asm volatile("" : "+v"(L[i]), "+v"(H[i]));
    }
}

enum { PR_NONE = 0, PR_OUT, PR_ZERO };
template <int NV> struct NarrowVar {
    static constexpr int NONE = 99;
    static constexpr int IFFT_FROM = NV == 0 ? NONE : (NV == 2 ? 1 : 0);
    static constexpr int FFT_FROM = NV == 0 ? NONE : (NV == 3 ? 1 : 0);
};

template <int P, int T, int NK, bool LB, int KB0, int KB1, bool FFT, bool IN_TAB2, int PRUNE, int G, class FIN = NoFin,
          class PRE = NoPre>
struct GroupLoop {
    static __device__ __forceinline__ void run(uint32_t (&L)[Geo<T>::NR], uint32_t (&H)[Geo<T>::NR], const Thr& c,
                                               const PassArgs& a, const uint4* tab1, const uint4* tab2,
                                               const uint32_t (&cur)[20], uint32_t zmask, const FIN& fin = FIN(),
                                               const PRE& pre = PRE()) {
        using S = LayerSeq<T, LB, KB0, KB1, FFT>;
        constexpr int s = S::step_of(G), gi = S::index_of(G);
        constexpr int kb = S::kb_of(s);
        constexpr int rb = kb - S::SH;
        constexpr bool more = G + 1 < S::total();
        constexpr bool NARROW = kb >= NK;
        uint32_t nxt[20];
        if constexpr (more)
            load_table_lds(nxt, group_table<T, LB, KB0, KB1, FFT, G + 1, IN_TAB2>(c, tab1, tab2));
        __builtin_amdgcn_sched_barrier(0);
        bool need = true;
        if constexpr (PRUNE == PR_OUT)
            need = ((uint32_t)gi << (kb + 1)) < a.need_hi && ((uint32_t)(gi + 1) << (kb + 1)) > a.need_lo;
        if constexpr (PRUNE == PR_ZERO) {
            static_assert(LB && kb >= 4, "zero pruning works on 16-row blocks of layout B");
            constexpr int nb = 1 << (kb - 3);
            constexpr uint32_t all = (uint32_t)((1ull << nb) - 1);
            need = ((zmask >> (gi * nb)) & all) != all;
        }
        bool mul = true;
        if constexpr (LB && gi == 0 && ProgTraits<P>::IFFT && ProgTraits<P>::FFT) {
            const uint32_t idx = (c.b_high << (a.lo + T)) + (1u << (a.lo + kb)) + (FFT ? a.skew_fft : a.skew_ifft) - 1;
            mul = (idx & (idx + 1)) != 0;
        }
        if (need && mul) {
#pragma unroll
            for (int j = 0; j < (1 << rb); j++) {
                const int m = (gi << (rb + 1)) + j, m2 = m + (1 << rb);
                if constexpr (!std::is_same<PRE, NoPre>::value && s == 0) pre(L, H, (gi << rb) + j);
                if (FFT) {
                    mul_xor_t<NARROW>(L[m], H[m], L[m2], H[m2], cur);
                    L[m2] ^= L[m];
                    H[m2] ^= H[m];
                } else {
                    L[m2] ^= L[m];
                    H[m2] ^= H[m];
                    mul_xor_t<NARROW>(L[m], H[m], L[m2], H[m2], cur);
                }
            }
        } else if (need) {
#pragma unroll
            for (int j = 0; j < (1 << rb); j++) {
                const int m = (gi << (rb + 1)) + j, m2 = m + (1 << rb);
                L[m2] ^= L[m];
                H[m2] ^= H[m];
            }
        }
#pragma unroll
        for (int j = 0; j < (1 << rb); j++) {
            const int m = (gi << (rb + 1)) + j, m2 = m + (1 << rb);
            asm volatile("" : "+v"(L[m]), "+v"(H[m]), "+v"(L[m2]), "+v"(H[m2]));
        }
        __builtin_amdgcn_sched_barrier(0);
        if constexpr (S::DF && kb == 0) fin(L, H, gi << 1);
        if constexpr (more)
            GroupLoop<P, T, NK, LB, KB0, KB1, FFT, IN_TAB2, PRUNE, G + 1, FIN, PRE>::run(L, H, c, a, tab1, tab2, nxt,
                                                                                          zmask, fin, pre);
    }
};

__device__ __forceinline__ const uint4* lds_vgpr(const uint4* p) {
    uint32_t v = (uint32_t)(uintptr_t)(const __attribute__((address_space(3))) uint4*)p;
    asm volatile("" : "+v"(v));
    return (const uint4*)(const __attribute__((address_space(3))) uint4*)(uintptr_t)v;
}

template <int P, int T, int NK, bool LB, int KB0, int KB1, bool FFT, bool IN_TAB2, int PRUNE = PR_NONE,
          class FIN = NoFin, class PRE = NoPre>
__device__ __forceinline__ void layers(uint32_t (&L)[Geo<T>::NR], uint32_t (&H)[Geo<T>::NR], const Thr& c,
                                       const PassArgs& a, const uint4* tab1, const uint4* tab2,
                                       uint32_t zmask = 0, const FIN& fin = FIN(), const PRE& pre = PRE()) {
    if constexpr (KB1 > KB0) {
        if constexpr (LB) {
            if constexpr (IN_TAB2) tab2 = lds_vgpr(tab2);
            else tab1 = lds_vgpr(tab1);
        }
        uint32_t t0[20];
        load_table_lds(t0, group_table<T, LB, KB0, KB1, FFT, 0, IN_TAB2>(c, tab1, tab2));
        GroupLoop<P, T, NK, LB, KB0, KB1, FFT, IN_TAB2, PRUNE, 0, FIN, PRE>::run(L, H, c, a, tab1, tab2, t0, zmask, fin,
                                                                                 pre);
    }
}

template <int T, int QL> struct Img {
    static constexpr int PLANE = (1 << T) * QL;
    static __device__ __forceinline__ uint32_t* at(uint2* lds, const Thr& c, uint32_t k) {
        return (uint32_t*)lds + k * QL + c.ql;
    }
};

template <int NQR> __device__ __forceinline__ bool my_round(const Thr& c, int r) {
    return NQR == 1 || c.round == (uint32_t)r;
}

template <int T, int QL, bool LB>
__device__ __forceinline__ void put_rows(const uint32_t (&L)[Geo<T>::NR], const uint32_t (&H)[Geo<T>::NR],
                                         const Thr& c, uint2* lds) {
#pragma unroll
    for (int m = 0; m < Geo<T>::NR; m++) {
        uint32_t* p = Img<T, QL>::at(lds, c, kidx<T, LB>(c, m));
        p[0] = L[m];
        p[Img<T, QL>::PLANE] = H[m];
    }
}
template <int T, int QL, bool LB>
__device__ __forceinline__ void get_rows(uint32_t (&L)[Geo<T>::NR], uint32_t (&H)[Geo<T>::NR], const Thr& c,
                                         uint2* lds) {
#pragma unroll
    for (int m = 0; m < Geo<T>::NR; m++) {
        const uint32_t* p = Img<T, QL>::at(lds, c, kidx<T, LB>(c, m));
        L[m] = p[0];
        H[m] = p[Img<T, QL>::PLANE];
    }
}

template <int T, int QL, bool LB>
__device__ __forceinline__ void fd_rows(uint32_t (&L)[Geo<T>::NR], uint32_t (&H)[Geo<T>::NR],
                                        const uint32_t (&SL)[Geo<T>::NR], const uint32_t (&SH)[Geo<T>::NR],
                                        const Thr& c, uint2* lds) {
    constexpr int R = Geo<T>::R, SHB = Geo<T>::SHB;
#pragma unroll
    for (int m = 0; m < Geo<T>::NR; m++) {
        const uint32_t k = kidx<T, LB>(c, m);
        uint32_t xl = L[m], xh = H[m];
#pragma unroll
        for (int b = 0; b < T; b++) {
            const bool reg_bit = LB ? (b >= SHB) : (b < R);
            if (reg_bit) {
                const int mb = LB ? b - SHB : b;
                if (!((m >> mb) & 1)) {
                    xl ^= SL[m | (1 << mb)];
                    xh ^= SH[m | (1 << mb)];
                }
            } else {
                constexpr int LOG_HWS = Geo<T>::HWS == 4 ? 2 : (Geo<T>::HWS == 2 ? 1 : 0);
                const int sb = LB ? b : b - R;
                if (sb >= LOG_HWS) {
                    if (!((c.w >> (sb - LOG_HWS)) & 1)) {
                        const uint32_t* p = Img<T, QL>::at(lds, c, k | (1u << b));
                        xl ^= p[0];
                        xh ^= p[Img<T, QL>::PLANE];
                    }
                } else {
                    const uint32_t* p = Img<T, QL>::at(lds, c, k | (1u << b));
                    const uint32_t vl = p[0], vh = p[Img<T, QL>::PLANE];
                    const bool take = !((k >> b) & 1);
                    xl ^= take ? vl : 0u;
                    xh ^= take ? vh : 0u;
                }
            }
        }
        L[m] = xl;
        H[m] = xh;
    }
}

struct NoMid {
    __device__ __forceinline__ void operator()() const {}
};
template <int T, int NQR, bool FROM_B, class MID = NoMid, class POST = NoMid>
__device__ __forceinline__ void exchange(uint32_t (&L)[Geo<T>::NR], uint32_t (&H)[Geo<T>::NR], const Thr& c,
                                         uint2* lds, MID mid = MID(), POST post = POST()) {
    constexpr int QL = Geo<T>::Q / NQR;
// ... 419 lines not shown
template <int P, int T, bool V32>
__device__ __forceinline__ void store_rows(const PassArgs& a, const Thr& cs, const uint32_t (&L)[Geo<T>::NR],
                                           const uint32_t (&H)[Geo<T>::NR], const uint4* rvt, const uint32_t* lostf) {
#pragma unroll
    for (int m = 0; m < Geo<T>::NR; m++) store_row<P, T, V32>(a, cs, L[m], H[m], m, rvt, lostf);
}
template <int P, int T, bool PAIR = false> struct EarlyStore {
    const PassArgs& a;
    const Thr& cs;
    const uint4* rvt;
    const uint32_t* lostf;
    const FastStore<P, T, PAIR> fs;
    __device__ __forceinline__ void operator()(const uint32_t (&L)[Geo<T>::NR], const uint32_t (&H)[Geo<T>::NR],
                                               int m) const {
        if (PAIR || fs.on) {
            fs.row(m, L[m], H[m]);
            fs.row(m + 1, L[m + 1], H[m + 1]);
        } else if (a.voff32) {
            store_row<P, T, true>(a, cs, L[m], H[m], m, rvt, lostf);
            store_row<P, T, true>(a, cs, L[m + 1], H[m + 1], m + 1, rvt, lostf);
        } else {
            store_row<P, T, false>(a, cs, L[m], H[m], m, rvt, lostf);
            store_row<P, T, false>(a, cs, L[m + 1], H[m + 1], m + 1, rvt, lostf);
        }
    }
};

template <int T> struct HalfSeq {
    static constexpr int SH = Geo<T>::SHB, NR = Geo<T>::NR;
    static constexpr int at(int g) {
        int n = 0;
        for (int half = 0; half < 2; half++)
            for (int kb = Geo<T>::R; kb < T; kb++) {
                const int rb = kb - SH;
                if (rb == 0 && half == 1) continue;
                for (int gi = 0; gi < (NR >> (rb + 1)); gi++)
                    if (n++ == g) return half * 256 + kb * 16 + gi;
            }
        return -1;
    }
    static constexpr int total() {
        int g = 0;
        while (at(g) >= 0) g++;
        return g;
    }
};
template <int T, int G, class FIN> struct HalfLoop {
    static __device__ __forceinline__ void run(uint32_t (&L)[Geo<T>::NR], uint32_t (&H)[Geo<T>::NR],
                                               const uint4* tab1, const uint32_t (&cur)[20], const FIN& fin) {
        using S = HalfSeq<T>;
        constexpr int e = S::at(G), half = e >> 8, kb = (e >> 4) & 15, gi = e & 15, rb = kb - S::SH;
        constexpr bool more = G + 1 < S::total();
        uint32_t nxt[20];
        if constexpr (more) {
            constexpr int kb2 = (S::at(G + 1) >> 4) & 15, gi2 = S::at(G + 1) & 15;
            load_table_lds(nxt, tab1 + ((1 << T) - (1 << (T - kb2)) + gi2) * 5);
        }
        __builtin_amdgcn_sched_barrier(0);
#pragma unroll
        for (int j = 0; j < (1 << rb); j++) {
            if (rb > 0 && (j & 1) != half) continue;
            const int m = (gi << (rb + 1)) + j, m2 = m + (1 << rb);
            L[m2] ^= L[m];
            H[m2] ^= H[m];
            mul_xor(L[m], H[m], L[m2], H[m2], cur);
            asm volatile("" : "+v"(L[m]), "+v"(H[m]), "+v"(L[m2]), "+v"(H[m2]));
        }
        __builtin_amdgcn_sched_barrier(0);
        if constexpr (more) {
            if constexpr (half == 0 && (S::at(G + 1) >> 8) == 1) fin(L, H);
            HalfLoop<T, G + 1, FIN>::run(L, H, tab1, nxt, fin);
        }
    }
};
template <int T, class FIN>
__device__ __forceinline__ void ifft_b_halves(uint32_t (&L)[Geo<T>::NR], uint32_t (&H)[Geo<T>::NR], const uint4* tab1,
                                              const FIN& fin) {
    constexpr int e = HalfSeq<T>::at(0), kb = (e >> 4) & 15, gi = e & 15;
    tab1 = lds_vgpr(tab1);
    uint32_t t0[20];
    load_table_lds(t0, tab1 + ((1 << T) - (1 << (T - kb)) + gi) * 5);
    HalfLoop<T, 0, FIN>::run(L, H, tab1, t0, fin);
}
template <int P, int T, bool PAIR = false> struct EvenStore {
    const PassArgs& a;
    const Thr& cs;
    const FastStore<P, T, PAIR> fs;
    __device__ __forceinline__ void operator()(const uint32_t (&L)[Geo<T>::NR], const uint32_t (&H)[Geo<T>::NR]) const {
        if (PAIR || fs.on) {
#pragma unroll
            for (int m = 0; m < Geo<T>::NR; m += 2) fs.row(m, L[m], H[m]);
            return;
        }
#pragma unroll
        for (int m = 0; m < Geo<T>::NR; m += 2) {
            if (a.voff32) store_row<P, T, true>(a, cs, L[m], H[m], m, nullptr, nullptr);
            else store_row<P, T, false>(a, cs, L[m], H[m], m, nullptr, nullptr);
        }
    }
};

template <int P, int T, int NV, class PRE = NoPre, bool PAIR_OUT = false>
__device__ __forceinline__ void process_item(const PassArgs& a, const Thr& c, uint32_t tile, ItemRegs<P, T>& d,
                                             uint8_t* smem, const PRE& pre = PRE()) {
    using PT = ProgTraits<P>;
    constexpr int NKI = NarrowVar<NV>::IFFT_FROM, NKF = NarrowVar<NV>::FFT_FROM;
    static_assert(NV == 0 || (PT::IFFT && PT::FFT && T > 4), "narrow variants: two-direction passes only");
    using SM = Smem<P, T>;
    using G = Geo<T>;
    constexpr int NR = G::NR;
    constexpr int R = G::R;
    constexpr int NQR = Rnd<P, T>::NQR;
    constexpr bool TWO = SM::TWO;
    constexpr bool ZERO_SKIP = P == DEC_MID && T > 4 && G::R == 4;
    constexpr bool EARLY = LayerSeq<T, false, 0, R, true>::DF && P != DEC_MID && PT::STORE != ST_RESTORE && PT::FFT &&
                           T > 4;
    constexpr bool EARLY_B = PT::IFFT && !PT::FFT && PT::STORE == ST_PLAIN && T > 4 && G::R == 4;
    uint2* lds = (uint2*)smem;
    const uint4* tab1 = (const uint4*)(smem + SM::TAB1_OFF);
    const uint4* tab2 = (const uint4*)(smem + SM::TAB2_OFF);
    const uint4* ert = (const uint4*)(smem + SM::ERT_OFF);
    const uint4* rvt = (const uint4*)(smem + SM::RVT_OFF);
    const uint32_t* lostf = (const uint32_t*)(smem + SM::LOST_OFF);
    uint32_t(&L)[NR] = d.L;
    uint32_t(&H)[NR] = d.H;
    constexpr bool START_B = !PT::IFFT;
    [[maybe_unused]] constexpr bool END_B = !PT::FFT && T > 4;
    constexpr bool SPLIT_FD = P == DEC_MID && T > 4;
    constexpr int FD_PB = 1 << (R - G::SHB);
    constexpr int FD_ND = FD_PB > 2 ? FD_PB : 2;
    [[maybe_unused]] bool fd_few = false;
    [[maybe_unused]] uint32_t fd_m0 = 0;
    [[maybe_unused]] uint32_t dl[FD_ND], dh[FD_ND];
    if constexpr (SPLIT_FD) {
        const uint32_t lo = uni(a.need_lo), hi = uni(min(a.need_hi, 1u << T));
        const uint32_t m0 = (lo >> R) * FD_PB, m1 = hi <= lo ? m0 : (((hi - 1) >> R) + 1) * FD_PB;
        fd_few = !a.fd_lds && m1 - m0 <= (uint32_t)FD_ND;
        fd_m0 = hi <= lo ? 0u : min(m0, (uint32_t)(NR - FD_ND));
    }

    if constexpr (P == DEC_FIRST) {
        if (a.zflags && tile_is_zero(a, tile)) {
            __builtin_amdgcn_s_waitcnt(vmcnt_wait(0));
            return;
        }
    }
    if constexpr (PT::LOAD == LD_GATHER_DEC) {
#pragma unroll
        for (int m = 0; m < NR; m++) {
            uint32_t tt[20];
            load_table_lds(tt, ert + kidx<T, START_B>(c, m) * 5);
            const uint32_t yl = L[m], yh = H[m];
            L[m] = H[m] = 0;
            mul_xor(L[m], H[m], yl, yh, tt);
        }
    }
    if constexpr (PT::LOAD == LD_DEC_LAST) {
        if (!d.ztile) tile_fd<T, NQR, START_B>(L, H, d.zl, d.zh, c, lds);
    }

    [[maybe_unused]] Stager<T, (SM::SHARED ? G::TSPLIT : 0)> s3s;
    bool in_b = START_B;
    if constexpr (PT::IFFT) {
        bool skip_a = false;
        if constexpr (ZERO_SKIP) skip_a = __all(d.zrow == (1u << NR) - 1);
        if constexpr (WaveStaged<P, T>::value) RS16_STAMP_ROWS(a, 6, L, H, 0, 1);
        if constexpr (!std::is_same<PRE, NoPre>::value)
            layers<P, T, NKI, false, 0, R, false, false, PR_NONE, NoFin, PRE>(L, H, c, a, tab1, tab2, 0, NoFin(), pre);
        else if (!skip_a) layers<P, T, NKI, false, 0, R, false, false>(L, H, c, a, tab1, tab2);
        RS16_STAMP(a, 3);
        prio<1>();
        if constexpr (T > 4) {
            constexpr bool LS2 = SM::RESTAGE && !SM::SHARED;
            Stager<T, (LS2 ? G::TSPLIT : 0)> s3;
            if constexpr (LS2) s3.issue(a.skew_tab, TwiddleEntry<T>{a, c, 0, a.skew_fft});
            if constexpr (SM::SHARED) __syncthreads();
            exchange<T, NQR, false>(
                L, H, c, lds,
                [&]() {
                    if constexpr (LS2) s3.commit((uint4*)(smem + SM::TAB1_OFF));
                },
                [&]() {
                    if constexpr (SPLIT_FD) {
                        if (fd_few) {
                            constexpr int QL = G::Q / NQR;
#pragma unroll
                            for (int i = 0; i < FD_ND; i++)
                                fd_image<T, QL>(dl[i], dh[i], c, lds, kidx<T, true>(c, fd_m0 + i));
                        }
                    }
                });
            RS16_STAMP(a, 4);
            if constexpr (SM::SHARED) s3s.issue(a.skew_tab, TwiddleEntry<T>{a, c, 0, a.skew_fft});
            if constexpr (EARLY_B) {
                Thr cs = c;
                asm volatile("" : "+v"(cs.offL));
                ifft_b_halves<T>(L, H, tab1, EvenStore<P, T, PAIR_OUT>{a, cs, FastStore<P, T, PAIR_OUT>(a, cs)});
            } else {
                const uint4* tab1b = SM::SHARED ? (const uint4*)(smem + SM::TABB_OFF) - G::TSPLIT * 5 : tab1;
                layers<P, T, NKI, true, R, (T > 4 ? T : R), false, false, (ZERO_SKIP ? PR_ZERO : PR_NONE)>(
                    L, H, c, a, tab1b, tab2, d.zmask);
            }
            in_b = true;
        }
        RS16_STAMP(a, 5);
        prio<2>();
    }
    if constexpr (PT::FD) {
        if constexpr (SPLIT_FD) {
            if (fd_few) fd_regs<T>(L, H);
            else tile_fd<T, NQR, true>(L, H, L, H, c, lds);
        } else {
            if (in_b) tile_fd<T, NQR, true>(L, H, L, H, c, lds);
            else tile_fd<T, NQR, false>(L, H, L, H, c, lds);
        }
        RS16_STAMP(a, 6);
    }
    if constexpr (PT::FFT) {
        if constexpr (T > 4) {
            if constexpr (WaveStaged<P, T>::value && !PT::IFFT) RS16_STAMP_ROWS(a, 6, L, H, 0, NR / 2);
            if constexpr (!std::is_same<PRE, NoPre>::value && !PT::IFFT)
                layers<P, T, NKF, true, R, T, true, TWO, PR_NONE, NoFin, PRE>(L, H, c, a, tab1, tab2, 0, NoFin(), pre);
            else
                layers<P, T, NKF, true, R, (T > 4 ? T : R), true, TWO, (P == DEC_MID ? PR_OUT : PR_NONE)>(L, H, c, a, tab1,
                                                                                                      tab2);
            if constexpr (SPLIT_FD) {
                if (fd_few) {
#pragma unroll
                    for (int m = 0; m < NR; m++) {
#pragma unroll
                        for (int i = 0; i < FD_ND; i++)
                            if ((uint32_t)m == fd_m0 + i) L[m] ^= dl[i], H[m] ^= dh[i];
                    }
                }
            }
            RS16_STAMP(a, 7);
            prio<3>();
            RevealStage<P, (LateReveal<P, T>::value ? T : 0)> rs;
            if constexpr (LateReveal<P, T>::value) {
                const uint32_t* el = nullptr;
                if (a.ework) {
                    const uint32_t base = a.row_base_out;
                    el = (const uint32_t*)(smem + SM::ELOG_OFF) + ((row_rel<T>(c, a, 0) + base) & 255u);
                }
                rs.issue(a, c, el);
            }
            if constexpr (SPLIT_FD) {
                if (fd_few) few_switch<T, FD_ND>(L, H, c, lds, fd_m0);
                else exchange<T, NQR, true>(L, H, c, lds);
            } else {
                exchange<T, NQR, true>(L, H, c, lds, [&]() {
                    if constexpr (LateReveal<P, T>::value) rs.commit(smem);
                });
            }
            if constexpr (SM::SHARED) {
                if constexpr (SPLIT_FD) {
                    if (fd_few) __syncthreads();
                }
                s3s.commit((uint4*)(smem + SM::TAB1_OFF));
                __syncthreads();
            }
            RS16_STAMP(a, 8);
            prio<4>();
            in_b = false;
        }
        bool need = true;
        if constexpr (P == DEC_MID) need = (c.s << R) < a.need_hi && ((c.s + 1) << R) > a.need_lo;
        if constexpr (PT::STORE == ST_RESTORE && T > 4) {
            uint32_t any = 0;
#pragma unroll
            for (int m = 0; m < NR; m++) any |= lostf[kidx<T, false>(c, m)];
            need = any != 0;
        }
        if constexpr (EARLY) {
            Thr cs = c;
            asm volatile("" : "+v"(cs.offL));
            layers<P, T, NKF, false, 0, R, true, (TWO && !(SM::RESTAGE))>(L, H, c, a, tab1, tab2, 0,
                                                                        EarlyStore<P, T, PAIR_OUT>{
                                                                            a, cs, rvt, lostf,
                                                                            FastStore<P, T, PAIR_OUT>(a, cs)});
        } else if (need) {
            layers<P, T, NKF, false, 0, R, true, (TWO && !(SM::RESTAGE))>(L, H, c, a, tab1, tab2);
        }
        RS16_STAMP(a, 9);
    }
    if constexpr (EARLY) {
        RS16_STAMP(a, 10);
        RS16_STAMP_END(a);
        return;
    }

    prio<5>();
    __builtin_amdgcn_s_waitcnt(vmcnt_wait(0));
    Thr cs = c;
    cs.b_low = uni(cs.b_low);
    cs.b_high = uni(cs.b_high);
    asm volatile("" : "+s"(cs.b_low), "+s"(cs.b_high));
    asm volatile("" : "+v"(cs.offL));
    const FastStore<P, T, PAIR_OUT> fs(a, cs);
    if (PAIR_OUT || fs.on) {
#pragma unroll
        for (int m = EARLY_B ? 1 : 0; m < NR; m += EARLY_B ? 2 : 1) fs.row(m, L[m], H[m]);
    } else if constexpr (EARLY_B) {
#pragma unroll
        for (int m = 1; m < NR; m += 2) {
            if (a.voff32) store_row<P, T, true>(a, cs, L[m], H[m], m, rvt, lostf);
            else store_row<P, T, false>(a, cs, L[m], H[m], m, rvt, lostf);
        }
    } else {
        if (a.voff32) store_rows<P, T, true>(a, cs, L, H, rvt, lostf);
        else store_rows<P, T, false>(a, cs, L, H, rvt, lostf);
    }
    RS16_STAMP(a, 10);
    RS16_STAMP_END(a);
}

template <int P, int T, int NV = 0>
__global__ void __launch_bounds__(Geo<T>::THREADS, ((P == DEC_SINGLE || P == DEC_HALF_SINGLE) ? 1 : 4))
    pass_kernel(PassArgs a) {
    using G = Geo<T>;
    extern __shared__ __attribute__((aligned(16))) uint8_t smem[];
    const uint32_t item = blockIdx.x;

    Thr c;
    c.lane = threadIdx.x & 63;
    c.w = uni(threadIdx.x >> 6);
    c.qt = c.lane % G::Q;
    c.s = c.w * G::HWS + c.lane / G::Q;
    c.ql = c.qt % Rnd<P, T>::QL;
    c.round = c.qt / Rnd<P, T>::QL;

    uint32_t tile, slab;
    set_item(c, a, item, G::Q, tile, slab);

    bool first_stripe = true;
    if (a.stripe_tiles) {
        const uint32_t st = uni(fast_div(tile, a.stripe_mul, a.stripe_one));
        first_stripe = st == 0;
        tile -= st * a.stripe_tiles;
        stripe_displace(a, st);
    }
    tile += a.tile_base;
    c.b_low = tile & ((1u << a.lo) - 1);
    c.b_high = tile >> a.lo;
    RcvCount<P, T> rcn;
    rcn.issue(a, c, slab == 0 && first_stripe);
    if constexpr (P == DEC_FIRST) {
        if (a.zflags && tile_is_zero(a, tile)) return;
    }
    if constexpr (P == DEC_MID) {
        uint32_t nlo, nhi;
        if (a.mid_direct && a.lostrange && mid_need(a, nlo, nhi)) return;
    }
    if constexpr (P == DEC_LAST) {
        if (a.lostrange) {
            const uint32_t r0 = ((cu32p)a.lostrange)[0], r1 = ((cu32p)a.lostrange)[1];
            if (!((tile << T) < r1 && ((tile + 1) << T) > r0)) return;
// ... 66 lines not shown
    if (a.stripe_tiles) {
        const uint32_t st = uni(fast_div(tile, a.stripe_mul, a.stripe_one));
        first_stripe = st == 0;
        tile -= st * a.stripe_tiles;
        stripe_displace(a, st);
    }
    tile += a.tile_base;
    c.b_low = tile & ((1u << a.lo) - 1);
    c.b_high = tile >> a.lo;
    RcvCount<P, T> rcn;
    rcn.issue(a, c, slab == 0 && first_stripe);
    RS16_STAMP(a, 0);
    const uint32_t slot = (__builtin_amdgcn_s_getreg((31 << 11) | 4) >> 16) & 15u;
    if (slot == 0) __builtin_amdgcn_s_setprio(3);
    else if (slot == 1) __builtin_amdgcn_s_setprio(2);
    else if (slot == 2) __builtin_amdgcn_s_setprio(1);
    TileStage<P, T> st;
    st.issue(a, c);
    ItemRegs<P, T> cur;
    cur.zrow = cur.zmask = 0;
    cur.ztile = false;
    const LateRows<P, T> rq(a, c);
    rq.prologue(cur.L, cur.H);
    RS16_STAMP(a, 1);
    prio<0>();
    st.template finish<false>(a, c, smem);
    rcn.count();
    RS16_STAMP(a, 2);
    process_item<P, T, NV, LateRows<P, T>>(a, c, tile, cur, smem, rq);
    rcn.store(a, c);
}
template <int P, int T, int NV, bool PAIR_IN, bool PAIR_OUT>
__global__ void __launch_bounds__(Geo<T>::THREADS, 4) pass_kernel_late_paired(PassArgs a) {
    static_assert(PAIR_IN || PAIR_OUT, "the unpaired kernel is pass_kernel_late");
    using G = Geo<T>;
    static_assert(WaveStaged<P, T>::value, "late rows: the wave-staged passes");
    extern __shared__ __attribute__((aligned(16))) uint8_t smem[];
    const uint32_t item = blockIdx.x;

    Thr c;
    c.lane = threadIdx.x & 63;
    c.w = uni(threadIdx.x >> 6);
    c.qt = c.lane % G::Q;
    c.s = c.w * G::HWS + c.lane / G::Q;
    c.ql = c.qt % Rnd<P, T>::QL;
    c.round = c.qt / Rnd<P, T>::QL;

    uint32_t tile, slab;
    set_item(c, a, item, G::Q, tile, slab);

    bool first_stripe = true;
    if (a.stripe_tiles) {
        const uint32_t st = uni(fast_div(tile, a.stripe_mul, a.stripe_one));
        first_stripe = st == 0;
        tile -= st * a.stripe_tiles;
        stripe_displace(a, st);
    }
    tile += a.tile_base;
    c.b_low = tile & ((1u << a.lo) - 1);
    c.b_high = tile >> a.lo;
    RcvCount<P, T> rcn;
    rcn.issue(a, c, slab == 0 && first_stripe);
    RS16_STAMP(a, 0);
    const uint32_t slot = (__builtin_amdgcn_s_getreg((31 << 11) | 4) >> 16) & 15u;
    if (slot == 0) __builtin_amdgcn_s_setprio(3);
    else if (slot == 1) __builtin_amdgcn_s_setprio(2);
    else if (slot == 2) __builtin_amdgcn_s_setprio(1);
    TileStage<P, T> st;
    st.issue(a, c);
    ItemRegs<P, T> cur;
    cur.zrow = cur.zmask = 0;
    cur.ztile = false;
    const LateRows<P, T, PAIR_IN> rq(a, c);
    rq.prologue(cur.L, cur.H);
    RS16_STAMP(a, 1);
    prio<0>();
    st.template finish<false>(a, c, smem);
    rcn.count();
    RS16_STAMP(a, 2);
    process_item<P, T, NV, LateRows<P, T, PAIR_IN>, PAIR_OUT>(a, c, tile, cur, smem, rq);
    rcn.store(a, c);
}

template <int P, int T, int NV> PassFn late_entry() {
    if constexpr (WaveStaged<P, T>::value) return pass_kernel_late<P, T, NV>;
    else return nullptr;
}
template <int P, int T, int NV = 0> PassFn paired_entry() {
    static_assert(P == ENC_FIRST || P == ENC_MID || P == ENC_LAST, "paired rows: the encoder's three passes");
    return pass_kernel_late_paired<P, T, NV, P != ENC_FIRST, P != ENC_LAST>;
}
template <int P, int T, int NV = 0> PassKernel pass_entry() {
    using PT = ProgTraits<P>;
    return {pass_kernel<P, T, NV>, Smem<P, T>::BYTES, Geo<T>::THREADS, Geo<T>::Q,
            !PT::IFFT ? Geo<T>::SHB : 0, (!PT::FFT && T > 4) ? Geo<T>::SHB : 0, Geo<T>::R,
            late_entry<P, T, NV>(), PT::LOAD == LD_GATHER_ENC ? 1 : 0};
}
template <int P> PassKernel pass_row(int T) {
    static const PassKernel row[9] = {pass_entry<P, 0>(), pass_entry<P, 1>(), pass_entry<P, 2>(),
                                      pass_entry<P, 3>(), pass_entry<P, 4>(), pass_entry<P, 5>(),
                                      pass_entry<P, 6>(), pass_entry<P, 7>(), pass_entry<P, 8>()};
    return row[T];
}
template <int P, int NV> PassKernel narrow_row(int T) {
    static const PassKernel row[4] = {pass_entry<P, 5, NV>(), pass_entry<P, 6, NV>(), pass_entry<P, 7, NV>(),
                                      pass_entry<P, 8, NV>()};
    return T >= 5 ? row[T - 5] : PassKernel{};
}

}
```

reed-solomon-16_amd/csrc/rs16_pass_common.hpp:

```cpp
#pragma once
#include "rs16_internal.hpp"

namespace rs16 {

typedef void (*PassFn)(PassArgs);
struct PassKernel {
    PassFn fn;
    int lds;
    int threads;
    int quads;
    int load_shb, store_shb;
    int reg_bits;
    PassFn late;
    int gather;
    PassFn paired = nullptr;
};
struct PassConsts {
    uint32_t nslab, voff32, full_lanes;
    uint64_t rs_in, rs_seg, rs_out;
    uint32_t late_rows;
};
PassConsts pass_launch_consts(const PassKernel& k, int T, const PassArgs& a);
const PassKernel& pass_kernel_of(int prog, int T);
constexpr int NARROW_VARIANTS = 4;
PassKernel pass_kernels_enc(int prog, int T, int nv);
PassKernel pass_kernels_dec(int prog, int T, int nv);

#if defined(__HIPCC__) || defined(__HIP__)
typedef const __attribute__((address_space(4))) uint32_t* cu32p;

__device__ __forceinline__ uint32_t uni(uint32_t v) { return __builtin_amdgcn_readfirstlane(v); }

__host__ __device__ constexpr int vmcnt_wait(int n) { return (n & 15) | ((n >> 4) << 14) | (7 << 4) | (15 << 8); }

__device__ __forceinline__ void load_table_lds(uint32_t (&t)[20], const uint4* p) {
#pragma unroll
    for (int i = 0; i < 5; i++) {
        const uint4 v = p[i];
        t[4 * i] = v.x;
        t[4 * i + 1] = v.y;
        t[4 * i + 2] = v.z;
        t[4 * i + 3] = v.w;
    }
}

__device__ __forceinline__ void stripe_displace(PassArgs& a, uint32_t st) {
    a.in += st * a.bs_in;
    a.in2 += st * a.bs_in2;
    a.out += st * a.bs_out;
    a.seg_a += st * a.bs_seg;
    a.seg_b += st * a.bs_seg_b;
    a.rest += st * a.bs_rest;
    if (a.flags_a) a.flags_a += st * a.bs_fa;
    if (a.flags_b) a.flags_b += st * a.bs_fb;
    if (a.elog) a.elog += st * a.bs_elog;
    if (a.ework) a.ework += st * a.bs_elog;
    if (a.rbits) a.rbits += st * a.bs_rbits;
    if (a.zflags) a.zflags += st * a.bs_zflags;
    if (a.lostrange) a.lostrange += st * a.bs_lost;
}

__device__ __forceinline__ bool tile_is_zero(const PassArgs& a, uint32_t tile) {
    return (((cu32p)a.zflags)[tile >> 2] >> (8 * (tile & 3))) & 1u;
}
__device__ __forceinline__ void lost_range(const PassArgs& a, uint32_t& r0, uint32_t& r1) {
    r0 = ((cu32p)a.lostrange)[0];
    r1 = ((cu32p)a.lostrange)[1];
}

template <int T> __device__ __forceinline__ bool tl_covers(const PassArgs& a) {
    uint32_t r0, r1;
    lost_range(a, r0, r1);
    return r0 < r1 && ((r1 - 1) >> T) - (r0 >> T) < a.tl_max;
}

__device__ __forceinline__ bool mid_need(const PassArgs& a, uint32_t& nlo, uint32_t& nhi) {
    uint32_t r0, r1;
    lost_range(a, r0, r1);
    if (r0 >= r1) return false;
    nlo = max(a.need_lo, r0 >> a.lo);
    nhi = min(a.need_hi, ((r1 - 1) >> a.lo) + 1);
    return nhi > nlo && nhi - nlo <= MID_DIRECT_MAX;
}

__device__ __forceinline__ bool row_lost_original(const PassArgs& a, uint32_t r) {
    const uint32_t base = a.rest_seg_b ? a.chunk : 0;
    const uint32_t cnt = a.rest_seg_b ? a.b_count : a.a_count;
    const uint8_t* fl = a.rest_seg_b ? a.flags_b : a.flags_a;
    return r >= base && r - base < cnt && fl && !fl[r - base];
}
#endif

}
```

reed-solomon-16_amd/csrc/rs16_pass_launch.hip:

```cpp
#include <algorithm>

#include "rs16_pass_common.hpp"

namespace rs16 {

struct KernelTable {
    PassKernel k[NUM_PROGS][9][NARROW_VARIANTS];
    KernelTable() {
        for (int prog = 0; prog < NUM_PROGS; prog++)
            for (int T = 0; T <= 8; T++)
                for (int nv = 0; nv < NARROW_VARIANTS; nv++) {
                    const PassKernel e = pass_kernels_enc(prog, T, nv);
                    k[prog][T][nv] = e.fn ? e : pass_kernels_dec(prog, T, nv);
                }
    }
};
static const PassKernel& find_kernel(int prog, int T, int nv) {
    static const KernelTable table;
    return table.k[prog][T][nv];
}

static const PassKernel& pick_kernel(int prog, int T, int ni, int nf) {
    for (int nv = 1; nv < NARROW_VARIANTS; nv++) {
        const int vi = nv == 2 ? 1 : 0, vf = nv == 3 ? 1 : 0;
        if (ni > vi || nf > vf) continue;
        const PassKernel& k = find_kernel(prog, T, nv);
        if (k.fn) return k;
    }
    return find_kernel(prog, T, 0);
}

const PassKernel& pass_kernel_of(int prog, int T) { return find_kernel(prog, T, 0); }

PassConsts pass_launch_consts(const PassKernel& k, int T, const PassArgs& a) {
    PassConsts c;
    c.nslab = (a.qrow + k.quads - 1) / k.quads;
    {
        const uint64_t hws = k.quads >= 64 ? 1 : 64 / k.quads;
        const uint64_t smax = std::max(std::max(a.S_in, a.S_out), std::max(a.S_seg, a.S_rest));
        const uint64_t span = (uint64_t)1 << (T + a.lo);
        const bool fits = (hws - 1) * ((uint64_t)16 << a.lo) * smax + 8 * (uint64_t)a.qrow <= ((uint64_t)1 << 32);
        const bool aligned = a.chunk % span == 0 && a.row_base_in % span == 0;
        c.voff32 = fits && aligned && !(a.diag & DIAG_FORCE_VOFF64) ? 1u : 0u;
    }
    c.rs_in = a.S_in << (a.lo + k.load_shb);
    c.rs_seg = a.S_seg << (a.lo + k.load_shb);
    c.rs_out = a.S_out << (a.lo + k.store_shb);
    const bool full = c.voff32 && a.qrow % k.quads == 0 && a.in_rows_mask == 0 && c.rs_out < ((uint64_t)1 << 28);
    c.full_lanes = full ? 1u : 0u;
    {
        const uint64_t hws = k.quads >= 64 ? 1 : 64 / k.quads;
        const uint64_t wave_span = (hws << k.reg_bits) << a.lo;
        const bool whole = !k.gather || a.a_count % wave_span == 0;
        const bool strides = c.rs_in < ((uint64_t)1 << 28) && c.rs_seg < ((uint64_t)1 << 28);
        c.late_rows = k.late && c.voff32 && a.in_rows_mask == 0 && whole && strides && !(a.diag & DIAG_NO_LATE_ROWS)
                          ? 1u
                          : 0u;
    }
    return c;
}

bool paired_rows_sequence(uint32_t chunk_rows, uint64_t S, uint64_t S_user, uint32_t a_count, uint32_t seg_chunk,
                          uint32_t row_base_in, int diag) {
    if (diag & DIAG_NO_PAIRED_ROWS) return false;
    if (chunk_rows < 512 || (chunk_rows & (chunk_rows - 1)) || S == 0 || S % 8 || S / 8 > 0xFFFFFFFFu) return false;
    int L = 0;
    while (((uint32_t)1 << L) < chunk_rows) L++;
    const int lo = L / 2, hi = L - lo;
    PassArgs a{};
    a.S_in = a.S_out = a.S_rest = S;
    a.S_seg = S_user;
    a.qrow = (uint32_t)(S / 8);
    a.a_count = a_count, a.chunk = seg_chunk, a.row_base_in = row_base_in;
    a.diag = (uint32_t)diag;
    const struct { int prog, T; uint32_t lo; uint64_t S_out; } seq[3] = {
        {ENC_FIRST, lo, 0, S}, {ENC_MID, hi, (uint32_t)lo, S}, {ENC_LAST, lo, 0, S_user}};
    for (const auto& p : seq) {
        if (p.T > 8) return false;
        const PassKernel& k = find_kernel(p.prog, p.T, 0);
        a.lo = p.lo, a.S_out = p.S_out;
        const PassConsts c = pass_launch_consts(k, p.T, a);
        if (!k.fn || !k.paired || !c.late_rows || !c.full_lanes) return false;
    }
    return true;
}

hipError_t launch_pass(int prog, int T, const PassArgs& args, uint32_t num_tiles, hipStream_t s) {
    if (prog < 0 || prog >= NUM_PROGS || T < 0 || T > 8) return hipErrorInvalidValue;
    if (num_tiles == 0 || args.qrow == 0) return hipSuccess;
    PassArgs a = args;
    int ni = T, nf = T;
    if (!(a.diag & DIAG_WIDE_TWIDDLES)) {
        const uint32_t bh_max = (a.tile_base + (a.stripe_tiles ? a.stripe_tiles : num_tiles) - 1) >> a.lo;
        ni = first_narrow_layer(a.lo, T, a.skew_ifft, bh_max);
        nf = first_narrow_layer(a.lo, T, a.skew_fft, bh_max);
    }
    const PassKernel& k = pick_kernel(prog, T, ni, nf);
    const PassConsts pc = pass_launch_consts(k, T, a);
    a.nslab = pc.nslab;
    a.ntiles = num_tiles;
    const uint32_t nwg = num_tiles * a.nslab;
    if (a.need_hi == 0) a.need_hi = 1u << T;
    a.voff32 = pc.voff32;
    a.fd_lds = (a.diag & DIAG_FD_LDS) ? 1u : 0u;
    a.rs_in = pc.rs_in, a.rs_seg = pc.rs_seg, a.rs_out = pc.rs_out;
    a.full_lanes = pc.full_lanes;
    const FastDiv dn = fast_div_of(a.nslab), ds = fast_div_of(a.stripe_tiles);
    a.nslab_mul = dn.mul, a.nslab_one = dn.one;
    a.stripe_mul = ds.mul, a.stripe_one = ds.one;
    const size_t lds = (size_t)k.lds;
    PassFn fn = pc.late_rows ? k.late : k.fn;
    if (a.paired) {
        if (a.paired != paired_sides_of(prog) || !k.paired || !pc.late_rows || !pc.full_lanes)
            return hipErrorInvalidValue;
        fn = k.paired;
    }
    if (lds > 65536) {
        hipError_t e = hipFuncSetAttribute((const void*)fn, hipFuncAttributeMaxDynamicSharedMemorySize, (int)lds);
        if (e != hipSuccess) return e;
    }
    dim3 grid(nwg), block(k.threads);
    hipLaunchKernelGGL(fn, grid, block, lds, s, a);
    return hipGetLastError();
}

}
```

reed-solomon-16_amd/csrc/rs16_tables.cpp:

```cpp
#include <cstdio>
#include <cstdlib>
#include <algorithm>
#include <cstring>
#include <mutex>
#include <vector>

#include "rs16_internal.hpp"

namespace rs16 {

namespace {
const uint16_t kCantorBasis[16] = {0x0001, 0xACCA, 0x3C0E, 0x163E, 0xC582, 0xED2E, 0x914C, 0x4012,
                                   0x6C98, 0x10D8, 0x6A72, 0xB900, 0xFDB8, 0xFB34, 0xFF38, 0x991E};
HostTables g_tables;
std::once_flag g_once;

inline uint16_t gf_mul(const HostTables& t, uint16_t x, uint32_t log_m) {
    return x == 0 ? 0 : t.exp[add_mod(t.log[x], log_m)];
}

void fwht_full(std::vector<uint16_t>& v) {
    for (uint32_t d = 1; d < GF_ORDER; d <<= 1)
        for (uint32_t r = 0; r < GF_ORDER; r += 2 * d)
            for (uint32_t i = r; i < r + d; i++) {
                uint32_t a = v[i], b = v[i + d];
                v[i] = (uint16_t)add_mod(a, b);
                v[i + d] = (uint16_t)sub_mod(a, b);
            }
}

void build(HostTables& t) {
    t.exp.assign(GF_ORDER, 0);
    t.log.assign(GF_ORDER, 0);
    {
        uint32_t state = 1;
        for (uint32_t i = 0; i < GF_MODULUS; i++) {
            t.exp[state] = (uint16_t)i;
            state <<= 1;
            if (state >= GF_ORDER) state ^= 0x1002Du;
        }
        t.exp[0] = (uint16_t)GF_MODULUS;
    }
    {
        std::vector<uint16_t> cb(GF_ORDER, 0);
        for (int b = 0; b < 16; b++) {
            uint32_t w = 1u << b;
            for (uint32_t j = 0; j < w; j++) cb[j + w] = cb[j] ^ kCantorBasis[b];
        }
        for (uint32_t i = 0; i < GF_ORDER; i++) t.log[i] = t.exp[cb[i]];
        for (uint32_t i = 0; i < GF_ORDER; i++) t.exp[t.log[i]] = (uint16_t)i;
        t.exp[GF_MODULUS] = t.exp[0];
    }
    {
        std::vector<uint16_t> sk(GF_MODULUS, 0);
        uint16_t temp[15];
        for (int i = 1; i < 16; i++) temp[i - 1] = (uint16_t)(1u << i);
        for (int m = 0; m < 15; m++) {
            const uint32_t step = 1u << (m + 1);
            sk[(1u << m) - 1] = 0;
            for (int i = m; i < 15; i++) {
                const uint32_t s = 1u << (i + 1);
                for (uint32_t j = (1u << m) - 1; j < s; j += step) sk[j + s] = sk[j] ^ temp[i];
            }
            temp[m] = (uint16_t)(GF_MODULUS - t.log[gf_mul(t, temp[m], t.log[temp[m] ^ 1])]);
            for (int i = m + 1; i < 15; i++) temp[i] = gf_mul(t, temp[i], add_mod(t.log[temp[i] ^ 1], temp[m]));
        }
        t.skew.resize(GF_MODULUS);
        for (uint32_t i = 0; i < GF_MODULUS; i++) t.skew[i] = t.log[sk[i]];
    }
    t.log_walsh = t.log;
    t.log_walsh[0] = 0;
    fwht_full(t.log_walsh);

    for (uint32_t i = 0; i < GF_MODULUS; i++)
        if ((t.skew[i] == GF_MODULUS) != ((i & (i + 1)) == 0)) {
            fprintf(stderr, "rs16: skew table sentinel at unexpected index %u\n", i);
            abort();
        }
    t.skew_entry.assign(GF_ORDER, ZERO_ENTRY);
    for (uint32_t i = 0; i < GF_MODULUS; i++) t.skew_entry[i] = t.skew[i] == GF_MODULUS ? ZERO_ENTRY : t.skew[i];

    t.mul_tab.assign((size_t)TAB_ENTRIES * TAB_DWORDS, 0);
    static const int kOff3[4] = {0, 3, 8, 11};
    static const int kOff2[2] = {6, 14};
    for (uint32_t lm = 0; lm < GF_ORDER; lm++) {
        uint32_t* e = &t.mul_tab[(size_t)lm * TAB_DWORDS];
        for (int g = 0; g < 4; g++)
            for (uint32_t v = 0; v < 8; v++) {
                uint16_t p = gf_mul(t, (uint16_t)(v << kOff3[g]), lm);
                for (int ob = 0; ob < 2; ob++) {
                    uint32_t byte = (p >> (8 * ob)) & 0xFF;
                    e[(g * 2 + ob) * 2 + (v >> 2)] |= byte << (8 * (v & 3));
                }
            }
        for (int gg = 0; gg < 2; gg++)
            for (uint32_t v = 0; v < 4; v++) {
                uint16_t p = gf_mul(t, (uint16_t)(v << kOff2[gg]), lm);
                for (int ob = 0; ob < 2; ob++) e[16 + gg * 2 + ob] |= ((p >> (8 * ob)) & 0xFFu) << (8 * v);
            }
    }

    t.skew_tab.resize((size_t)GF_ORDER * TAB_DWORDS);
    for (uint32_t i = 0; i < GF_ORDER; i++)
        std::copy_n(&t.mul_tab[(size_t)t.skew_entry[i] * TAB_DWORDS], TAB_DWORDS, &t.skew_tab[(size_t)i * TAB_DWORDS]);
    for (uint32_t i = 0; i < GF_MODULUS; i++) {
        const uint32_t* e = &t.skew_tab[(size_t)i * TAB_DWORDS];
        const bool zero = (e[2] | e[3] | e[6] | e[7] | e[17]) == 0;
        if (zero != twiddle_narrow(i)) {
            fprintf(stderr, "rs16: skew table entry %u is %s a subfield twiddle, against the index rule\n", i,
                    zero ? "" : "not");
            abort();
        }
    }

    t.col_img.assign(COL_IMG_DWORDS, 0);
    for (uint32_t L = COL_LMIN; L <= COL_LGEN; L++)
        for (uint32_t d = 0; d < col_img_count(L); d++) {
            const uint32_t N = 1u << L, delta = d * N;
            uint32_t* img = &t.col_img[col_img_offset(L, d)];
            for (uint32_t g = 0; g + 1 < N; g++) {
                uint32_t kb = 0;
                while (g >= N - (N >> (kb + 1))) kb++;
                const uint32_t j = g - (N - (N >> kb));
                const uint32_t idx = (j << (kb + 1)) + (1u << kb) + delta - 1;
                std::copy_n(&t.skew_tab[(size_t)idx * TAB_DWORDS], 20, img + (size_t)g * 20);
            }
        }

    {
        std::vector<int64_t> w(GF_ORDER);
        for (uint32_t i = 0; i < GF_ORDER; i++) w[i] = t.log_walsh[i];
        auto fwht = [](int64_t* x, uint32_t n) {
            for (uint32_t d = 1; d < n; d <<= 1)
                for (uint32_t i = 0; i < n; i += 2 * d)
                    for (uint32_t j = i; j < i + d; j++) {
                        const int64_t a = x[j], b = x[j + d];
                        x[j] = a + b;
                        x[j + d] = a - b;
                    }
        };
        auto mod = [](int64_t v) { return (uint32_t)(((v % 65535) + 65535) % 65535); };
        fwht(w.data(), GF_ORDER);
        t.col_k.assign(COL_LGEN + 2, 0);
        {
            int64_t pre = 0;
            for (uint32_t n = 1, j = 0; n <= (2u << COL_LMAX); n <<= 1) {
                for (; j < n; j++) pre += mod(w[j]);
                uint32_t lg = 0;
                while ((1u << lg) < n) lg++;
                if (lg < t.col_k.size()) t.col_k[lg] = mod((int64_t)t.log_walsh[0] - pre);
            }
        }
        t.col_v.assign(COL_V_DWORDS, 0);
        for (uint32_t n = 1u << COL_LMIN; n <= (2u << COL_LMAX); n <<= 1) {
            std::vector<int64_t> v(n);
            for (uint32_t i = 0; i < n; i++) v[i] = mod(w[i]);
            fwht(v.data(), n);
            uint32_t lg = 0;
            while ((1u << lg) < n) lg++;
            const int64_t inv = (int64_t)1 << (16 - lg);
            for (uint32_t k = 0; k < n; k++) t.col_v[col_v_offset(n) + k] = mod(mod(v[k]) * inv);
        }
    }
}
}

std::vector<uint32_t> mid_matrix_entries(const HostTables& t, int L) {
    const int lo = L / 2, hi = L - lo;
    const uint32_t N = 1u << hi;
    const uint16_t one = t.exp[0];
    std::vector<uint32_t> ent((size_t)N * N, ZERO_ENTRY);
    std::vector<uint16_t> v(N), w(N);
    auto tw = [&](uint32_t r_tile, int kb) {
        const uint32_t m = (uint32_t)(lo + kb);
        return (uint32_t)t.skew[((size_t)r_tile << lo) + (1u << m) - 1];
    };
    for (uint32_t c = 0; c < N; c++) {
        std::fill(v.begin(), v.end(), 0);
        v[c] = one;
        for (int kb = 0; kb < hi; kb++) {
            const uint32_t d = 1u << kb;
            for (uint32_t r = 0; r < N; r += 2 * d) {
                const uint32_t lm = tw(r, kb);
                for (uint32_t i = r; i < r + d; i++) {
                    v[i + d] ^= v[i];
                    if (lm != GF_MODULUS) v[i] ^= gf_mul(t, v[i + d], lm);
                }
            }
        }
        for (uint32_t i = 0; i < N; i++) {
            uint16_t x = v[i];
            for (uint32_t b = 1; b < N; b <<= 1)
                if (!(i & b)) x ^= v[i | b];
            w[i] = x;
        }
        for (int kb = hi - 1; kb >= 0; kb--) {
// ... 21 lines not shown
```

reed-solomon-16_amd/rs16/__init__.py:

```python
from __future__ import annotations

import atexit
import ctypes as C
import weakref
from typing import Iterable, Iterator, Optional, Tuple

import numpy as np

from ._lib import RS16Error, lib

__all__ = [
    "Error", "Engine", "default_engine", "ReedSolomonEncoder", "ReedSolomonDecoder", "RateEncoder",
    "RateDecoder", "EncoderResult", "DecoderResult", "encode", "decode", "encode_device", "decode_device",
    "supports", "validate", "use_high_rate", "encode_device_batch", "decode_device_batch", "encoder_work_count", "decoder_work_count",
    "RATE_DEFAULT", "RATE_HIGH", "RATE_LOW", "GF_ORDER", "GF_MODULUS", "set_diagnostics",
    "DIAG_FORCE_VOFF64", "DIAG_EVAL_TWO_KERNEL", "DIAG_EVAL_FULL", "DIAG_NO_COLUMN", "DIAG_FORCE_COLUMN",
    "DIAG_TILE_LAST", "DIAG_NO_TILE_LAST", "DIAG_FD_LDS", "DIAG_COL_RADIX4", "DIAG_NO_IDENTITY", "DIAG_NO_MID_DIRECT", "DIAG_WIDE_TWIDDLES", "DIAG_NO_LATE_ROWS", "DIAG_NO_PAIRED_ROWS", "encode_host", "decode_host",
    "encode_host_batch", "decode_host_batch", "decode_prepare", "decode_device_prepared",
    "UpdatePlan", "update_recovery_device", "UPDATE_MAX_SHARDS",
    "encode_host_multi", "decode_host_multi", "Comm", "column_slice", "scatter_columns", "gather_columns",
]

GF_ORDER = 65536
GF_MODULUS = 65535
DIAG_FORCE_VOFF64, DIAG_EVAL_TWO_KERNEL, DIAG_EVAL_FULL, DIAG_NO_COLUMN, DIAG_FORCE_COLUMN = 1, 2, 4, 8, 16
DIAG_TILE_LAST, DIAG_NO_TILE_LAST, DIAG_FD_LDS, DIAG_COL_RADIX4, DIAG_NO_IDENTITY = 32, 64, 128, 256, 512
DIAG_NO_MID_DIRECT = 1024
DIAG_WIDE_TWIDDLES = 2048
DIAG_NO_LATE_ROWS = 4096
DIAG_NO_PAIRED_ROWS = 8192
_diag_default = 0


def set_diagnostics(flags: int, engine: Optional["Engine"] = None) -> int:
    global _diag_default
    if engine is not None:
        return engine.set_diagnostics(flags)
    old, _diag_default = _diag_default, flags
    for e in list(_live_engines):
        if getattr(e, "h", None):
            e.set_diagnostics(flags)
    return old
RATE_DEFAULT, RATE_HIGH, RATE_LOW = 0, 1, 2
_RATES = {"default": 0, "high": 1, "low": 2, 0: 0, 1: 1, 2: 2}

_VARIANTS = {
    1: ("DifferentShardSize", ("shard_bytes", "got")),
    2: ("DuplicateOriginalShardIndex", ("index",)),
    3: ("DuplicateRecoveryShardIndex", ("index",)),
    4: ("InvalidOriginalShardIndex", ("original_count", "index")),
    5: ("InvalidRecoveryShardIndex", ("recovery_count", "index")),
    6: ("InvalidShardSize", ("shard_bytes",)),
    7: ("NotEnoughShards", ("original_count", "original_received_count", "recovery_received_count")),
    8: ("TooFewOriginalShards", ("original_count", "original_received_count")),
    9: ("TooManyOriginalShards", ("original_count",)),
    10: ("UnsupportedShardCount", ("original_count", "recovery_count")),
    100: ("DeviceError", ("hip_error",)),
    101: ("InvalidArgument", ()),
}
_CODES = {name: code for code, (name, _) in _VARIANTS.items()}


class Error(Exception):

    def __init__(self, kind: str, **fields):
        if kind not in _CODES:
            raise ValueError(kind)
        self.kind, self.fields = kind, fields
        self.code = _CODES[kind]
        super().__init__(self._message())

    @classmethod
    def _from_c(cls, e: RS16Error) -> "Error":
        name, fnames = _VARIANTS.get(e.code, ("InvalidArgument", ()))
        vals = (e.v0, e.v1, e.v2)
        err = cls(name, **{f: int(v) for f, v in zip(fnames, vals)})
        return err

    def _message(self) -> str:
        e = RS16Error(self.code, 0, 0, 0)
        vals = list(self.fields.values()) + [0, 0, 0]
        e.v0, e.v1, e.v2 = vals[0], vals[1], vals[2]
        buf = C.create_string_buffer(256)
        lib().rs16_error_message(C.byref(e), buf, 256)
        return buf.value.decode()

    def __eq__(self, other):
        return isinstance(other, Error) and (self.kind, self.fields) == (other.kind, other.fields)

    def __hash__(self):
        return hash((self.kind, tuple(sorted(self.fields.items()))))

    def __repr__(self):
        return f"Error.{self.kind}({', '.join(f'{k}={v}' for k, v in self.fields.items())})"


def _check(rc: int, err: RS16Error):
    if rc != 0:
        raise Error._from_c(err)


def _is_device(x) -> bool:
    return bool(getattr(x, "is_cuda", False))


def _device_ptr_len(x) -> Tuple[int, int]:
    if not x.is_contiguous():
        raise ValueError("device shard must be contiguous")
    return x.data_ptr(), x.numel() * x.element_size()


def _host_buf(x):
    if isinstance(x, np.ndarray):
# ... 729 lines not shown
```

reed-solomon-16_amd/rs16/_lib.py:

```python
from __future__ import annotations

import ctypes as C
import os
from pathlib import Path

PKG_ROOT = Path(__file__).resolve().parents[1]
LIB_PATH = Path(os.environ.get("RS16_LIB", PKG_ROOT / "build" / "librs16.so"))


class RS16Error(C.Structure):
    _fields_ = [("code", C.c_int32), ("v0", C.c_uint64), ("v1", C.c_uint64), ("v2", C.c_uint64)]


class PassConsts(C.Structure):
    _fields_ = [(n, C.c_uint32) for n in ("voff32", "full_lanes", "nslab", "quads", "threads", "load_shb",
                                          "store_shb", "reg_bits", "row_sets")] + \
               [(n, C.c_uint64) for n in ("rs_in", "rs_seg", "rs_out")] + [("late_rows", C.c_uint32)]


_sz, _p, _i, _e = C.c_size_t, C.c_void_p, C.c_int, C.POINTER(RS16Error)
_u32, _u64 = C.c_uint32, C.c_uint64

SIGNATURES = {
    "rs16_error_message": (_sz, [_e, C.c_char_p, _sz]),
    "rs16_version": (C.c_char_p, []),
    "rs16_host_mul": (None, [_p, _p, _sz, C.c_uint16]),
    "rs16_host_mul_narrow": (None, [_p, _p, _sz, C.c_uint16]),
    "rs16_host_twiddle": (C.c_uint32, [C.c_uint32, C.POINTER(C.c_uint32), C.POINTER(C.c_uint32)]),
    "rs16_host_twiddle_narrow": (C.c_int, [C.c_uint32]),
    "rs16_host_fast_div_check": (C.c_uint64, [C.c_uint32, C.c_uint32, C.c_uint32, C.c_uint32]),
    "rs16_host_pass_consts": (_i, [_i, _i, _u32, _u64, _u64, _u64, _u64, _u32, _u32, _u32, _u32, _i,
                                   C.POINTER(PassConsts)]),
    "rs16_host_pass_consts_rows": (_i, [_i, _i, _u32, _u64, _u64, _u64, _u64, _u32, _u32, _u32, _u32, _u32, _i,
                                        C.POINTER(PassConsts)]),
    "rs16_host_pass_consts_many": (_i, [_i, _i, _u32, _sz, _p, _p, _p, _p, _p, _u32, _u32, _u32, _i, _p]),
    "rs16_host_paired_rows": (_i, [_u32, _u64, _u64, _u32, _u32, _u32, _i]),
    "rs16_host_update_consts": (_i, [_u32, _u64, _u32, C.POINTER(_u32), C.POINTER(_u32), C.POINTER(_u32),
                                     C.POINTER(_u64)]),
    "rs16_engine_set_profiling": (_i, [_p, _i, _e]),
    "rs16_engine_profile_read": (_i, [_p, _i, C.POINTER(C.c_double), C.POINTER(C.c_uint64), _e]),
    "rs16_engine_profile_reset": (None, [_p]),
    "rs16_prog_count": (_i, []),
    "rs16_engine_set_diagnostics": (_i, [_p, _i]),
    "rs16_prog_name": (C.c_char_p, [_i]),
    "rs16_engine_set_stamps": (_i, [_p, _p, _i, _e]),
    "rs16_engine_set_slices": (_i, [_p, _i, _e]),
    "rs16_engine_new": (_p, [_i, _e]),
    "rs16_engine_new_ex": (_p, [_i, _i, _e]),
    "rs16_set_diagnostics": (_i, [_i]),
    "rs16_engine_free": (None, [_p]),
    "rs16_engine_device": (_i, [_p]),
    "rs16_engine_stream": (_p, [_p]),
    "rs16_engine_synchronize": (_i, [_p, _p, _e]),
    "rs16_engine_fft": (_i, [_p, _p, _sz, _sz, _sz, _sz, _sz, _sz, _p, _e]),
    "rs16_engine_fft_skew_end": (_i, [_p, _p, _sz, _sz, _sz, _sz, _sz, _p, _e]),
    "rs16_engine_ifft": (_i, [_p, _p, _sz, _sz, _sz, _sz, _sz, _sz, _p, _e]),
    "rs16_engine_ifft_skew_end": (_i, [_p, _p, _sz, _sz, _sz, _sz, _sz, _p, _e]),
    "rs16_engine_fwht": (_i, [_p, _p, _sz, _p, _e]),
    "rs16_engine_eval_poly": (_i, [_p, _p, _sz, _p, _e]),
    "rs16_engine_mul": (_i, [_p, _p, _sz, C.c_uint16, _p, _e]),
    "rs16_engine_xor": (_i, [_p, _p, _p, _sz, _p, _e]),
    "rs16_engine_xor_within": (_i, [_p, _p, _sz, _sz, _sz, _sz, _sz, _p, _e]),
    "rs16_engine_formal_derivative": (_i, [_p, _p, _sz, _sz, _p, _e]),
    "rs16_supports": (_i, [_i, _sz, _sz]),
    "rs16_validate": (_i, [_i, _sz, _sz, _sz, _e]),
    "rs16_use_high_rate": (_i, [_sz, _sz, _e]),
    "rs16_encoder_work_count": (_sz, [_i, _sz, _sz]),
    "rs16_decoder_work_count": (_sz, [_i, _sz, _sz]),
    "rs16_encoder_new": (_p, [_p, _i, _sz, _sz, _sz, _e]),
    "rs16_encoder_free": (None, [_p]),
    "rs16_encoder_reset": (_i, [_p, _sz, _sz, _sz, _e]),
    "rs16_encoder_add_original_shard": (_i, [_p, _p, _sz, _e]),
    "rs16_encoder_add_original_shard_device": (_i, [_p, _p, _sz, _e]),
    "rs16_encoder_encode": (_i, [_p, _e]),
    "rs16_encoder_recovery": (_p, [_p, _sz, _e]),
    "rs16_encoder_recovery_device": (_p, [_p, _sz]),
    "rs16_encoder_recovery_copy": (_i, [_p, _sz, _p, _sz, _e]),
    "rs16_encoder_result_drop": (None, [_p]),
    "rs16_encoder_is_high_rate": (_i, [_p]),
    "rs16_decoder_new": (_p, [_p, _i, _sz, _sz, _sz, _e]),
    "rs16_decoder_free": (None, [_p]),
    "rs16_decoder_reset": (_i, [_p, _sz, _sz, _sz, _e]),
    "rs16_decoder_add_original_shard": (_i, [_p, _sz, _p, _sz, _e]),
    "rs16_decoder_add_recovery_shard": (_i, [_p, _sz, _p, _sz, _e]),
    "rs16_decoder_add_original_shard_device": (_i, [_p, _sz, _p, _sz, _e]),
    "rs16_decoder_add_recovery_shard_device": (_i, [_p, _sz, _p, _sz, _e]),
    "rs16_decoder_decode": (_i, [_p, _e]),
    "rs16_decoder_restored_original": (_p, [_p, _sz, _e]),
    "rs16_decoder_restored_original_device": (_p, [_p, _sz]),
    "rs16_decoder_restored_original_copy": (_i, [_p, _sz, _p, _sz, _e]),
    "rs16_decoder_result_drop": (None, [_p]),
    "rs16_decoder_is_high_rate": (_i, [_p]),
    "rs16_encode_device": (_i, [_p, _sz, _sz, _sz, _p, _p, _p, _e]),
    "rs16_encode_device_batch": (_i, [_p, _sz, _sz, _sz, _sz, _p, _sz, _p, _sz, _p, _e]),
    "rs16_decode_device_batch": (_i, [_p, _sz, _sz, _sz, _sz, _p, _sz, _p, _p, _sz, _p, _sz, _sz, _p, _e]),
    "rs16_decode_device_batch_varied": (_i, [_p, _sz, _sz, _sz, _sz, _p, _sz, _p, _sz, _p, _sz, _p, _sz, _p, _p, _p,
                                             _e]),
    "rs16_decode_device": (_i, [_p, _sz, _sz, _sz, _p, _p, _p, _p, _sz, _sz, _p, _e]),
    "rs16_decode_check": (_i, [_p, _p, _e]),
    "rs16_device_alloc": (_p, [_p, _sz, _e]),
    "rs16_device_free": (None, [_p, _p]),
    "rs16_memcpy_htod": (_i, [_p, _p, _p, _sz, _p, _e]),
    "rs16_memcpy_dtoh": (_i, [_p, _p, _p, _sz, _p, _e]),
    "rs16_memset_device": (_i, [_p, _p, _i, _sz, _p, _e]),
    "rs16_memcpy2d_htod": (_i, [_p, _p, _sz, _p, _sz, _sz, _sz, _p, _e]),
    "rs16_memcpy2d_dtoh": (_i, [_p, _p, _sz, _p, _sz, _sz, _sz, _p, _e]),
    "rs16_encode_host": (_i, [_p, _sz, _sz, _sz, _p, _p, _sz, _e]),
    "rs16_decode_host": (_i, [_p, _sz, _sz, _sz, _p, _p, _p, _p, _sz, _e]),
    "rs16_host_alloc": (_p, [_p, _sz, _e]),
    "rs16_comm_unique_id": (_i, [_p, _e]),
    "rs16_comm_new": (_p, [_p, _i, _i, _p, _e]),
    "rs16_comm_init_all": (_i, [_p, _i, _p, _e]),
    "rs16_comm_free": (None, [_p]),
    "rs16_comm_rank": (_i, [_p]),
    "rs16_comm_size": (_i, [_p]),
    "rs16_column_slice": (_i, [_sz, _i, _i, C.POINTER(_sz), C.POINTER(_sz)]),
    "rs16_scatter_columns": (_i, [_p, _i, _i, _sz, _sz, _p, _p, _p, _e]),
    "rs16_gather_columns": (_i, [_p, _i, _i, _sz, _sz, _p, _p, _p, _e]),
    "rs16_scatter_columns_virtual": (_i, [_p, _i, _sz, _sz, _p, _p, _p, _e]),
# ... 42 lines not shown
```

Before: 1074 GiB/s.

## Add tower-field basis for mid FFT pass to use cheaper subfield twiddle multiplies

Introduces a tower-field (GF(2^8)-over-GF(2^8)) basis change for the paired-rows encode/decode path. The first pass's output and the last pass's input are converted with a small per-element basis transform, so the middle pass can use twiddle tables in tower representation. In that representation, subfield twiddles use a narrow multiply with fewer permute lookups and no cross-byte terms. This cuts ALU work in the middle FFT pass, at the cost of extra conversion arithmetic in the first and last passes and a second device twiddle table.

```diff
diff --git a/include/rs16.h b/include/rs16.h
--- a/include/rs16.h
+++ b/include/rs16.h
@@ -214,7 +214,8 @@
     RS16_DIAG_NO_MID_DIRECT = 1024,
     RS16_DIAG_WIDE_TWIDDLES = 2048,
     RS16_DIAG_NO_LATE_ROWS = 4096,
-    RS16_DIAG_NO_PAIRED_ROWS = 8192
+    RS16_DIAG_NO_PAIRED_ROWS = 8192,
+    RS16_DIAG_NO_TOWER_ROWS = 16384
 };
 int rs16_engine_set_diagnostics(rs16_engine* eng, int flags);
 int rs16_set_diagnostics(int flags);
@@ -241,6 +242,12 @@
                                uint32_t in_rows_mask, uint32_t a_count, int diag, rs16_pass_consts* out);
 int rs16_host_paired_rows(uint32_t chunk_rows, uint64_t S, uint64_t S_user, uint32_t a_count, uint32_t seg_chunk,
                           uint32_t row_base_in, int diag);
+int rs16_host_tower_rows(uint32_t chunk_rows, uint64_t S, uint64_t S_user, uint32_t a_count, uint32_t seg_chunk,
+                         uint32_t row_base_in, int diag);
+uint32_t rs16_host_tower_basis(uint32_t i);
+void rs16_host_tower_conv(const void* in, void* out, size_t bytes);
+int rs16_host_tower_twiddle(uint32_t index, uint32_t* table20);
+void rs16_host_mul_tower(const void* in, void* out, size_t bytes, uint32_t index, int narrow);
 int rs16_host_update_consts(uint32_t rows, uint64_t shard_bytes, uint32_t n, uint32_t* quads_per_lane,
                             uint32_t* nslab, uint32_t* rows_per_wave, uint64_t* blocks);
 
diff --git a/reed-solomon-16_amd/csrc/rs16_api.cpp b/reed-solomon-16_amd/csrc/rs16_api.cpp
--- a/reed-solomon-16_amd/csrc/rs16_api.cpp
+++ b/reed-solomon-16_amd/csrc/rs16_api.cpp
@@ -57,8 +57,7 @@
     return n;
 }
 
-template <class Mul> static void host_mul(const void* in, void* out, size_t bytes, uint16_t log_m, Mul mul) {
-    const uint32_t* t = &host_tables().mul_tab[(size_t)log_m * TAB_DWORDS];
+template <class F> static void host_mul_table(const void* in, void* out, size_t bytes, const uint32_t* t, F mul) {
     const uint8_t* src = (const uint8_t*)in;
     uint8_t* dst = (uint8_t*)out;
     for (size_t q = 0; q < bytes / 8; q++) {
@@ -70,6 +69,9 @@
         memcpy(dst + off, &ol, 4);
         memcpy(dst + off + 32, &oh, 4);
     }
+}
+template <class Mul> static void host_mul(const void* in, void* out, size_t bytes, uint16_t log_m, Mul mul) {
+    host_mul_table(in, out, bytes, &host_tables().mul_tab[(size_t)log_m * TAB_DWORDS], mul);
 }
 extern "C" void rs16_host_mul(const void* in, void* out, size_t bytes, uint16_t log_m) {
     host_mul(in, out, bytes, log_m, mul_xor);
@@ -140,6 +142,35 @@
                                      uint32_t seg_chunk, uint32_t row_base_in, int diag) {
     return paired_rows_sequence(chunk_rows, S, S_user, a_count, seg_chunk, row_base_in, diag) ? 1 : 0;
 }
+extern "C" int rs16_host_tower_rows(uint32_t chunk_rows, uint64_t S, uint64_t S_user, uint32_t a_count,
+                                    uint32_t seg_chunk, uint32_t row_base_in, int diag) {
+    return tower_rows_sequence(chunk_rows, S, S_user, a_count, seg_chunk, row_base_in, diag) ? 1 : 0;
+}
+extern "C" uint32_t rs16_host_tower_basis(uint32_t i) { return i < 8 ? host_tables().tower_a[i] : ~0u; }
+extern "C" void rs16_host_tower_conv(const void* in, void* out, size_t bytes) {
+    TowerB tb;
+    memcpy(tb.p, host_tables().tower_b, sizeof tb.p);
+    const uint8_t* src = (const uint8_t*)in;
+    uint8_t* dst = (uint8_t*)out;
+    for (size_t q = 0; q < bytes / 8; q++) {
+        const size_t off = (q >> 3) * 64 + (q & 7) * 4;
+        uint32_t l, h;
+        memcpy(&l, src + off, 4);
+        memcpy(&h, src + off + 32, 4);
+        tower_conv(l, h, tb);
+        memcpy(dst + off, &l, 4);
+        memcpy(dst + off + 32, &h, 4);
+    }
+}
+extern "C" int rs16_host_tower_twiddle(uint32_t index, uint32_t* table20) {
+    if (index >= GF_MODULUS) return 0;
+    if (table20) memcpy(table20, &host_tables().skew_tab_tower[(size_t)index * TAB_DWORDS], 20 * sizeof(uint32_t));
+    return 1;
+}
+extern "C" void rs16_host_mul_tower(const void* in, void* out, size_t bytes, uint32_t index, int narrow) {
+    const uint32_t* t = &host_tables().skew_tab_tower[(size_t)(index < GF_MODULUS ? index : GF_MODULUS) * TAB_DWORDS];
+    host_mul_table(in, out, bytes, t, narrow ? mul_xor_tower_narrow : mul_xor);
+}
 extern "C" int rs16_host_update_consts(uint32_t rows, uint64_t shard_bytes, uint32_t n, uint32_t* quads_per_lane,
                                        uint32_t* nslab, uint32_t* rows_per_wave, uint64_t* blocks) {
     if (shard_bytes == 0 || (shard_bytes & 63) != 0 || shard_bytes / 8 > 0xFFFFFFFFu) return 0;
@@ -211,7 +242,7 @@
 static constexpr int DIAG_ALL = DIAG_FORCE_VOFF64 | DIAG_EVAL_TWO_KERNEL | DIAG_EVAL_FULL | DIAG_NO_COLUMN |
                                 DIAG_FORCE_COLUMN | DIAG_TILE_LAST | DIAG_NO_TILE_LAST | DIAG_FD_LDS |
                                 DIAG_COL_RADIX4 | DIAG_NO_IDENTITY | DIAG_NO_MID_DIRECT | DIAG_WIDE_TWIDDLES |
-                                DIAG_NO_LATE_ROWS | DIAG_NO_PAIRED_ROWS;
+                                DIAG_NO_LATE_ROWS | DIAG_NO_PAIRED_ROWS | DIAG_NO_TOWER_ROWS;
 extern "C" int rs16_engine_set_diagnostics(rs16_engine* e, int flags) {
     const int old = e->diag;
     e->diag = flags & DIAG_ALL;
@@ -319,11 +350,13 @@
     }
     e->flags = flags;
     if ((he = hipMalloc(&e->d_skew_tab, (size_t)GF_ORDER * TAB_DWORDS * 4)) != hipSuccess) return fail(he);
+    if ((he = hipMalloc(&e->d_skew_tab_tower, (size_t)GF_ORDER * TAB_DWORDS * 4)) != hipSuccess) return fail(he);
     if ((he = hipMalloc(&e->d_mul_tab, t.mul_tab.size() * 4)) != hipSuccess) return fail(he);
     if ((he = hipMalloc(&e->d_log_walsh, GF_ORDER * 2)) != hipSuccess) return fail(he);
     if ((he = hipMalloc(&e->d_zero_sink, RS16_ZERO_BYTES)) != hipSuccess) return fail(he);
     if ((he = hipMemset(e->d_zero_sink, 0, RS16_ZERO_BYTES)) != hipSuccess) return fail(he);
     if ((he = hipMemcpy(e->d_skew_tab, t.skew_tab.data(), t.skew_tab.size() * 4, hipMemcpyHostToDevice)) != hipSuccess) return fail(he);
+    if ((he = hipMemcpy(e->d_skew_tab_tower, t.skew_tab_tower.data(), t.skew_tab_tower.size() * 4, hipMemcpyHostToDevice)) != hipSuccess) return fail(he);
     if ((he = hipMemcpy(e->d_mul_tab, t.mul_tab.data(), t.mul_tab.size() * 4, hipMemcpyHostToDevice)) != hipSuccess) return fail(he);
     if ((he = hipMemcpy(e->d_log_walsh, t.log_walsh.data(), GF_ORDER * 2, hipMemcpyHostToDevice)) != hipSuccess) return fail(he);
     set_error(err, RS16_OK);
@@ -367,6 +400,7 @@
     }
     if (e->sl_fork) (void)hipEventDestroy(e->sl_fork);
     if (e->d_skew_tab) (void)hipFree(e->d_skew_tab);
+    if (e->d_skew_tab_tower) (void)hipFree(e->d_skew_tab_tower);
     if (e->d_mul_tab) (void)hipFree(e->d_mul_tab);
     if (e->d_col_img) (void)hipFree(e->d_col_img);
     if (e->d_col_v) (void)hipFree(e->d_col_v);
diff --git a/reed-solomon-16_amd/csrc/rs16_engine.cpp b/reed-solomon-16_amd/csrc/rs16_engine.cpp
--- a/reed-solomon-16_amd/csrc/rs16_engine.cpp
+++ b/reed-solomon-16_amd/csrc/rs16_engine.cpp
@@ -371,19 +371,23 @@
     const int lo = L / 2, hi = L - lo;
     const size_t zs = chunk * S;
     const bool paired = paired_rows_sequence((uint32_t)chunk, S, S_user, a.a_count, a.chunk, a.row_base_in, diag);
+    const uint32_t tower =
+        tower_rows_sequence((uint32_t)chunk, S, S_user, a.a_count, a.chunk, a.row_base_in, diag) ? PAIRED_TOWER : 0;
     a.out = Z;
     a.lo = 0;
-    a.paired = paired ? paired_sides_of(ENC_FIRST) : 0;
+    a.paired = paired ? paired_sides_of(ENC_FIRST) | tower : 0;
     RS16_PASS(ENC_FIRST, lo, a, batch(1u << hi, 0, zs, bs_orig), s);
     a.in = Z;
     a.lo = lo;
-    a.paired = paired ? paired_sides_of(ENC_MID) : 0;
+    a.paired = paired ? paired_sides_of(ENC_MID) | tower : 0;
+    if (tower) a.skew_tab = d_skew_tab_tower;
     RS16_PASS(ENC_MID, hi, a, batch(1u << lo, zs, zs, 0), s);
+    a.skew_tab = d_skew_tab;
     a.in = Z;
     a.out = d_rec;
     a.S_out = S_user;
     a.lo = 0;
-    a.paired = paired ? paired_sides_of(ENC_LAST) : 0;
+    a.paired = paired ? paired_sides_of(ENC_LAST) | tower : 0;
     const uint32_t tiles = (uint32_t)((m + ((size_t)1 << lo) - 1) >> lo);
     RS16_PASS(ENC_LAST, lo, a, batch(tiles, zs, bs_rec, 0), s);
     return RS16_OK;
@@ -561,20 +565,24 @@
             a.cnt_base = src;
             a.cnt_seg = g.high ? 0 : 1;
             const bool paired = paired_rows_sequence(half, S, S_user, a.a_count, a.chunk, a.row_base_in, diag);
+            const uint32_t tower =
+                tower_rows_sequence(half, S, S_user, a.a_count, a.chunk, a.row_base_in, diag) ? PAIRED_TOWER : 0;
             a.lo = 0;
             a.out = Z;
-            a.paired = paired ? paired_sides_of(ENC_FIRST) : 0;
+            a.paired = paired ? paired_sides_of(ENC_FIRST) | tower : 0;
             RS16_PASS_AS(PROF_DEC_HALF_FIRST, ENC_FIRST, lo, a, batch(1u << hi, 0, 0, zs), s);
             a.rcount = nullptr;
             a.lo = lo;
             a.in = Z;
-            a.paired = paired ? paired_sides_of(ENC_MID) : 0;
+            a.paired = paired ? paired_sides_of(ENC_MID) | tower : 0;
+            if (tower) a.skew_tab = d_skew_tab_tower;
             RS16_PASS_AS(PROF_DEC_HALF_MID, ENC_MID, hi, a, batch(1u << lo, zs, 0, zs), s);
+            a.skew_tab = d_skew_tab;
             a.lo = 0;
             a.out = rest;
             a.S_out = S_user;
             a.out_rows = orig;
-            a.paired = paired ? paired_sides_of(ENC_LAST) : 0;
+            a.paired = paired ? paired_sides_of(ENC_LAST) | tower : 0;
             a.rcount = rcount;
             a.cnt_flags = g.high ? flags_b : flags_a;
             a.cnt_base = dst;
diff --git a/reed-solomon-16_amd/csrc/rs16_engine.hpp b/reed-solomon-16_amd/csrc/rs16_engine.hpp
--- a/reed-solomon-16_amd/csrc/rs16_engine.hpp
+++ b/reed-solomon-16_amd/csrc/rs16_engine.hpp
@@ -66,6 +66,7 @@
     hipStream_t stream = nullptr;
     int diag = 0;
     uint32_t* d_skew_tab = nullptr;
+    uint32_t* d_skew_tab_tower = nullptr;
     uint32_t* d_mul_tab = nullptr;
     uint32_t* d_col_img = nullptr;
     uint32_t* d_col_v = nullptr;
diff --git a/reed-solomon-16_amd/csrc/rs16_gf.hpp b/reed-solomon-16_amd/csrc/rs16_gf.hpp
--- a/reed-solomon-16_amd/csrc/rs16_gf.hpp
+++ b/reed-solomon-16_amd/csrc/rs16_gf.hpp
@@ -99,6 +99,36 @@
     mul_xor_t<true>(xL, xH, yL, yH, t);
 }
 
+constexpr uint32_t TOWER_B_DWORD = 20;
+struct TowerB {
+    uint32_t p[5];
+};
+RS16_HD void tower_conv_sel(uint32_t& L, const MulSel& y, const TowerB& tb) {
+    const uint32_t b0 = perm(tb.p[1], tb.p[0], y.s3);
+    const uint32_t b1 = perm(tb.p[3], tb.p[2], y.s4);
+    const uint32_t b2 = perm(tb.p[4], tb.p[4], y.s5);
+    L = xor3(L, b0, b1) ^ b2;
+}
+RS16_HD MulSel high_selectors(uint32_t H) {
+    const uint32_t a = H >> 3;
+    return MulSel{0, 0, 0, H & 0x07070707u, a & 0x07070707u, (a >> 3) & 0x03030303u};
+}
+RS16_HD void tower_conv(uint32_t& L, uint32_t H, const TowerB& tb) { tower_conv_sel(L, high_selectors(H), tb); }
+RS16_HD MulSel low_selectors(uint32_t L, const MulSel& y) {
+    const uint32_t a = L >> 3;
+    return MulSel{L & 0x07070707u, a & 0x07070707u, (a >> 3) & 0x03030303u, y.s3, y.s4, y.s5};
+}
+RS16_HD void mul_xor_tower_narrow_sel(uint32_t& xL, uint32_t& xH, const MulSel& y, const uint32_t* t) {
+    const uint32_t l0 = perm(t[1], t[0], y.s0), h0 = perm(t[1], t[0], y.s3);
+    const uint32_t l1 = perm(t[5], t[4], y.s1), h1 = perm(t[5], t[4], y.s4);
+    const uint32_t l2 = perm(t[16], t[16], y.s2), h2 = perm(t[16], t[16], y.s5);
+    xL = xor3(xL, l0, l1) ^ l2;
+    xH = xor3(xH, h0, h1) ^ h2;
+}
+RS16_HD void mul_xor_tower_narrow(uint32_t& xL, uint32_t& xH, uint32_t yL, uint32_t yH, const uint32_t* t) {
+    mul_xor_tower_narrow_sel(xL, xH, mul_selectors(yL, yH), t);
+}
+
 RS16_HD uint32_t add_mod(uint32_t x, uint32_t y) {
     uint32_t s = x + y;
     return (s + (s >> 16)) & 0xFFFFu;
diff --git a/reed-solomon-16_amd/csrc/rs16_internal.hpp b/reed-solomon-16_amd/csrc/rs16_internal.hpp
--- a/reed-solomon-16_amd/csrc/rs16_internal.hpp
+++ b/reed-solomon-16_amd/csrc/rs16_internal.hpp
@@ -14,6 +14,9 @@
     std::vector<uint32_t> skew_entry;
     std::vector<uint32_t> mul_tab;
     std::vector<uint32_t> skew_tab;
+    uint8_t tower_a[8] = {};
+    uint32_t tower_b[5] = {};
+    std::vector<uint32_t> skew_tab_tower;
     std::vector<uint32_t> col_img;
     std::vector<uint32_t> col_v;
     std::vector<uint32_t> col_k;
@@ -196,6 +199,7 @@
     DIAG_WIDE_TWIDDLES = 2048,
     DIAG_NO_LATE_ROWS = 4096,
     DIAG_NO_PAIRED_ROWS = 8192,
+    DIAG_NO_TOWER_ROWS = 16384,
 };
 
 constexpr size_t RS16_ZERO_BYTES = 65536;
@@ -203,7 +207,9 @@
 hipError_t launch_pass(int prog, int T, const PassArgs& a, uint32_t num_tiles, hipStream_t s);
 bool paired_rows_sequence(uint32_t chunk_rows, uint64_t S, uint64_t S_user, uint32_t a_count, uint32_t seg_chunk,
                           uint32_t row_base_in, int diag);
-enum PairedSides : uint32_t { PAIRED_IN = 1, PAIRED_OUT = 2 };
+enum PairedSides : uint32_t { PAIRED_IN = 1, PAIRED_OUT = 2, PAIRED_TOWER = 4 };
+bool tower_rows_sequence(uint32_t chunk_rows, uint64_t S, uint64_t S_user, uint32_t a_count, uint32_t seg_chunk,
+                         uint32_t row_base_in, int diag);
 inline uint32_t paired_sides_of(int prog) {
     return prog == ENC_FIRST ? PAIRED_OUT : prog == ENC_MID ? PAIRED_IN | PAIRED_OUT : prog == ENC_LAST ? PAIRED_IN : 0u;
 }
diff --git a/reed-solomon-16_amd/csrc/rs16_pass.hpp b/reed-solomon-16_amd/csrc/rs16_pass.hpp
--- a/reed-solomon-16_amd/csrc/rs16_pass.hpp
+++ b/reed-solomon-16_amd/csrc/rs16_pass.hpp
@@ -472,7 +472,7 @@
 };
 
 template <int P, int T, int NK, bool LB, int KB0, int KB1, bool FFT, bool IN_TAB2, int PRUNE, int G, class FIN = NoFin,
-          class PRE = NoPre>
+          class PRE = NoPre, bool TW = false>
 struct GroupLoop {
     static __device__ __forceinline__ void run(uint32_t (&L)[Geo<T>::NR], uint32_t (&H)[Geo<T>::NR], const Thr& c,
                                                const PassArgs& a, const uint4* tab1, const uint4* tab2,
@@ -507,7 +507,25 @@
             for (int j = 0; j < (1 << rb); j++) {
                 const int m = (gi << (rb + 1)) + j, m2 = m + (1 << rb);
                 if constexpr (!std::is_same<PRE, NoPre>::value && s == 0) pre(L, H, (gi << rb) + j);
-                if (FFT) {
+                if constexpr (TW && P == ENC_LAST && LB && FFT && s == 0) {
+                    MulSel y = high_selectors(H[m2]);
+                    tower_conv_sel(L[m2], y, pre.tb);
+                    y = low_selectors(L[m2], y);
+                    tower_conv(L[m], H[m], pre.tb);
+                    mul_xor_sel<false>(L[m], H[m], y, cur);
+                    L[m2] ^= L[m];
+                    H[m2] ^= H[m];
+                } else if constexpr (TW && P == ENC_MID && NARROW) {
+                    if (FFT) {
+                        mul_xor_tower_narrow(L[m], H[m], L[m2], H[m2], cur);
+                        L[m2] ^= L[m];
+                        H[m2] ^= H[m];
+                    } else {
+                        L[m2] ^= L[m];
+                        H[m2] ^= H[m];
+                        mul_xor_tower_narrow(L[m], H[m], L[m2], H[m2], cur);
+                    }
+                } else if (FFT) {
                     mul_xor_t<NARROW>(L[m], H[m], L[m2], H[m2], cur);
                     L[m2] ^= L[m];
                     H[m2] ^= H[m];
@@ -533,8 +551,8 @@
         __builtin_amdgcn_sched_barrier(0);
         if constexpr (S::DF && kb == 0) fin(L, H, gi << 1);
         if constexpr (more)
-            GroupLoop<P, T, NK, LB, KB0, KB1, FFT, IN_TAB2, PRUNE, G + 1, FIN, PRE>::run(L, H, c, a, tab1, tab2, nxt,
-                                                                                          zmask, fin, pre);
+            GroupLoop<P, T, NK, LB, KB0, KB1, FFT, IN_TAB2, PRUNE, G + 1, FIN, PRE, TW>::run(L, H, c, a, tab1, tab2,
+                                                                                              nxt, zmask, fin, pre);
     }
 };
 
@@ -545,7 +563,7 @@
 }
 
 template <int P, int T, int NK, bool LB, int KB0, int KB1, bool FFT, bool IN_TAB2, int PRUNE = PR_NONE,
-          class FIN = NoFin, class PRE = NoPre>
+          class FIN = NoFin, class PRE = NoPre, bool TW = false>
 __device__ __forceinline__ void layers(uint32_t (&L)[Geo<T>::NR], uint32_t (&H)[Geo<T>::NR], const Thr& c,
                                        const PassArgs& a, const uint4* tab1, const uint4* tab2,
                                        uint32_t zmask = 0, const FIN& fin = FIN(), const PRE& pre = PRE()) {
@@ -556,8 +574,8 @@
         }
         uint32_t t0[20];
         load_table_lds(t0, group_table<T, LB, KB0, KB1, FFT, 0, IN_TAB2>(c, tab1, tab2));
-        GroupLoop<P, T, NK, LB, KB0, KB1, FFT, IN_TAB2, PRUNE, 0, FIN, PRE>::run(L, H, c, a, tab1, tab2, t0, zmask, fin,
-                                                                                 pre);
+        GroupLoop<P, T, NK, LB, KB0, KB1, FFT, IN_TAB2, PRUNE, 0, FIN, PRE, TW>::run(L, H, c, a, tab1, tab2, t0, zmask,
+                                                                                     fin, pre);
     }
 }
 
@@ -1143,6 +1161,52 @@
     load_table_lds(t0, tab1 + ((1 << T) - (1 << (T - kb)) + gi) * 5);
     HalfLoop<T, 0, FIN>::run(L, H, tab1, t0, fin);
 }
+template <int T, int G, class FIN> struct HalfLoopTower {
+    static __device__ __forceinline__ void run(uint32_t (&L)[Geo<T>::NR], uint32_t (&H)[Geo<T>::NR],
+                                               const uint4* tab1, const uint32_t (&cur)[20], const FIN& fin,
+                                               const TowerB& tb) {
+        using S = HalfSeq<T>;
+        constexpr int e = S::at(G), half = e >> 8, kb = (e >> 4) & 15, gi = e & 15, rb = kb - S::SH;
+        constexpr bool more = G + 1 < S::total();
+        uint32_t nxt[20];
+        if constexpr (more) {
+            constexpr int kb2 = (S::at(G + 1) >> 4) & 15, gi2 = S::at(G + 1) & 15;
+            load_table_lds(nxt, tab1 + ((1 << T) - (1 << (T - kb2)) + gi2) * 5);
+        }
+        __builtin_amdgcn_sched_barrier(0);
+#pragma unroll
+        for (int j = 0; j < (1 << rb); j++) {
+            if (rb > 0 && (j & 1) != half) continue;
+            const int m = (gi << (rb + 1)) + j, m2 = m + (1 << rb);
+            L[m2] ^= L[m];
+            H[m2] ^= H[m];
+            if constexpr (kb == T - 1) {
+                const MulSel y = mul_selectors(L[m2], H[m2]);
+                mul_xor_sel<false>(L[m], H[m], y, cur);
+                tower_conv_sel(L[m2], y, tb);
+                tower_conv(L[m], H[m], tb);
+            } else {
+                mul_xor(L[m], H[m], L[m2], H[m2], cur);
+            }
+            asm volatile("" : "+v"(L[m]), "+v"(H[m]), "+v"(L[m2]), "+v"(H[m2]));
+        }
+        __builtin_amdgcn_sched_barrier(0);
+        if constexpr (more) {
+            if constexpr (half == 0 && (S::at(G + 1) >> 8) == 1) fin(L, H);
+            HalfLoopTower<T, G + 1, FIN>::run(L, H, tab1, nxt, fin, tb);
+        }
+    }
+};
+template <int T, class FIN>
+__device__ __forceinline__ void ifft_b_halves_tower(uint32_t (&L)[Geo<T>::NR], uint32_t (&H)[Geo<T>::NR],
+                                                    const uint4* tab1, const FIN& fin, const TowerB& tb) {
+    static_assert(HalfSeq<T>::SH < Geo<T>::R, "every row's last layer is kb = T - 1, in its own half");
+    constexpr int e = HalfSeq<T>::at(0), kb = (e >> 4) & 15, gi = e & 15;
+    tab1 = lds_vgpr(tab1);
+    uint32_t t0[20];
+    load_table_lds(t0, tab1 + ((1 << T) - (1 << (T - kb)) + gi) * 5);
+    HalfLoopTower<T, 0, FIN>::run(L, H, tab1, t0, fin, tb);
+}
 template <int P, int T, bool PAIR = false> struct EvenStore {
     const PassArgs& a;
     const Thr& cs;
@@ -1161,7 +1225,7 @@
     }
 };
 
-template <int P, int T, int NV, class PRE = NoPre, bool PAIR_OUT = false>
+template <int P, int T, int NV, class PRE = NoPre, bool PAIR_OUT = false, bool TOWER = false>
 __device__ __forceinline__ void process_item(const PassArgs& a, const Thr& c, uint32_t tile, ItemRegs<P, T>& d,
                                              uint8_t* smem, const PRE& pre = PRE()) {
     using PT = ProgTraits<P>;
@@ -1227,7 +1291,8 @@
         if constexpr (ZERO_SKIP) skip_a = __all(d.zrow == (1u << NR) - 1);
         if constexpr (WaveStaged<P, T>::value) RS16_STAMP_ROWS(a, 6, L, H, 0, 1);
         if constexpr (!std::is_same<PRE, NoPre>::value)
-            layers<P, T, NKI, false, 0, R, false, false, PR_NONE, NoFin, PRE>(L, H, c, a, tab1, tab2, 0, NoFin(), pre);
+            layers<P, T, NKI, false, 0, R, false, false, PR_NONE, NoFin, PRE, TOWER>(L, H, c, a, tab1, tab2, 0, NoFin(),
+                                                                                     pre);
         else if (!skip_a) layers<P, T, NKI, false, 0, R, false, false>(L, H, c, a, tab1, tab2);
         RS16_STAMP(a, 3);
         prio<1>();
@@ -1256,7 +1321,14 @@
             if constexpr (EARLY_B) {
                 Thr cs = c;
                 asm volatile("" : "+v"(cs.offL));
-                ifft_b_halves<T>(L, H, tab1, EvenStore<P, T, PAIR_OUT>{a, cs, FastStore<P, T, PAIR_OUT>(a, cs)});
+                if constexpr (TOWER)
+                    ifft_b_halves_tower<T>(L, H, tab1, EvenStore<P, T, PAIR_OUT>{a, cs, FastStore<P, T, PAIR_OUT>(a, cs)},
+                                           pre.tb);
+                else
+                    ifft_b_halves<T>(L, H, tab1, EvenStore<P, T, PAIR_OUT>{a, cs, FastStore<P, T, PAIR_OUT>(a, cs)});
+            } else if constexpr (TOWER) {
+                const uint4* tab1b = SM::SHARED ? (const uint4*)(smem + SM::TABB_OFF) - G::TSPLIT * 5 : tab1;
+                layers<P, T, NKI, true, R, T, false, false, PR_NONE, NoFin, NoPre, true>(L, H, c, a, tab1b, tab2);
             } else {
                 const uint4* tab1b = SM::SHARED ? (const uint4*)(smem + SM::TABB_OFF) - G::TSPLIT * 5 : tab1;
                 layers<P, T, NKI, true, R, (T > 4 ? T : R), false, false, (ZERO_SKIP ? PR_ZERO : PR_NONE)>(
@@ -1281,7 +1353,10 @@
         if constexpr (T > 4) {
             if constexpr (WaveStaged<P, T>::value && !PT::IFFT) RS16_STAMP_ROWS(a, 6, L, H, 0, NR / 2);
             if constexpr (!std::is_same<PRE, NoPre>::value && !PT::IFFT)
-                layers<P, T, NKF, true, R, T, true, TWO, PR_NONE, NoFin, PRE>(L, H, c, a, tab1, tab2, 0, NoFin(), pre);
+                layers<P, T, NKF, true, R, T, true, TWO, PR_NONE, NoFin, PRE, TOWER>(L, H, c, a, tab1, tab2, 0, NoFin(),
+                                                                                     pre);
+            else if constexpr (TOWER)
+                layers<P, T, NKF, true, R, T, true, TWO, PR_NONE, NoFin, NoPre, true>(L, H, c, a, tab1, tab2);
             else
                 layers<P, T, NKF, true, R, (T > 4 ? T : R), true, TWO, (P == DEC_MID ? PR_OUT : PR_NONE)>(L, H, c, a, tab1,
                                                                                                       tab2);
@@ -1333,7 +1408,13 @@
             for (int m = 0; m < NR; m++) any |= lostf[kidx<T, false>(c, m)];
             need = any != 0;
         }
-        if constexpr (EARLY) {
+        if constexpr (EARLY && TOWER) {
+            Thr cs = c;
+            asm volatile("" : "+v"(cs.offL));
+            layers<P, T, NKF, false, 0, R, true, (TWO && !(SM::RESTAGE)), PR_NONE, EarlyStore<P, T, PAIR_OUT>, NoPre,
+                   true>(L, H, c, a, tab1, tab2, 0,
+                         EarlyStore<P, T, PAIR_OUT>{a, cs, rvt, lostf, FastStore<P, T, PAIR_OUT>(a, cs)});
+        } else if constexpr (EARLY) {
             Thr cs = c;
             asm volatile("" : "+v"(cs.offL));
             layers<P, T, NKF, false, 0, R, true, (TWO && !(SM::RESTAGE))>(L, H, c, a, tab1, tab2, 0,
@@ -1566,6 +1647,66 @@
     rcn.store(a, c);
 }
 
+template <int P, int T, bool PAIR> struct LateRowsTower : LateRows<P, T, PAIR> {
+    TowerB tb;
+    __device__ __forceinline__ LateRowsTower(const PassArgs& a, const Thr& c) : LateRows<P, T, PAIR>(a, c) {
+        const cu32p q = (cu32p)a.skew_tab + TOWER_B_DWORD;
+#pragma unroll
+        for (int i = 0; i < 5; i++) tb.p[i] = q[i];
+    }
+};
+template <int P, int T, int NV> __global__ void __launch_bounds__(Geo<T>::THREADS, 4) pass_kernel_late_tower(PassArgs a) {
+    static_assert(P == ENC_FIRST || P == ENC_MID || P == ENC_LAST, "tower rows: the encoder's three passes");
+    constexpr bool PAIR_IN = P != ENC_FIRST, PAIR_OUT = P != ENC_LAST;
+    using G = Geo<T>;
+    using RQ = typename std::conditional<P == ENC_MID, LateRows<P, T, PAIR_IN>, LateRowsTower<P, T, PAIR_IN>>::type;
+    extern __shared__ __attribute__((aligned(16))) uint8_t smem[];
+    const uint32_t item = blockIdx.x;
+
+    Thr c;
+    c.lane = threadIdx.x & 63;
+    c.w = uni(threadIdx.x >> 6);
+    c.qt = c.lane % G::Q;
+    c.s = c.w * G::HWS + c.lane / G::Q;
+    c.ql = c.qt % Rnd<P, T>::QL;
+    c.round = c.qt / Rnd<P, T>::QL;
+
+    uint32_t tile, slab;
+    set_item(c, a, item, G::Q, tile, slab);
+
+    bool first_stripe = true;
+    if (a.stripe_tiles) {
+        const uint32_t st = uni(fast_div(tile, a.stripe_mul, a.stripe_one));
+        first_stripe = st == 0;
+        tile -= st * a.stripe_tiles;
+        stripe_displace(a, st);
+    }
+    tile += a.tile_base;
+    c.b_low = tile & ((1u << a.lo) - 1);
+    c.b_high = tile >> a.lo;
+    RcvCount<P, T> rcn;
+    rcn.issue(a, c, slab == 0 && first_stripe);
+    RS16_STAMP(a, 0);
+    const uint32_t slot = (__builtin_amdgcn_s_getreg((31 << 11) | 4) >> 16) & 15u;
+    if (slot == 0) __builtin_amdgcn_s_setprio(3);
+    else if (slot == 1) __builtin_amdgcn_s_setprio(2);
+    else if (slot == 2) __builtin_amdgcn_s_setprio(1);
+    TileStage<P, T> st;
+    st.issue(a, c);
+    ItemRegs<P, T> cur;
+    cur.zrow = cur.zmask = 0;
+    cur.ztile = false;
+    const RQ rq(a, c);
+    rq.prologue(cur.L, cur.H);
+    RS16_STAMP(a, 1);
+    prio<0>();
+    st.template finish<false>(a, c, smem);
+    rcn.count();
+    RS16_STAMP(a, 2);
+    process_item<P, T, NV, RQ, PAIR_OUT, true>(a, c, tile, cur, smem, rq);
+    rcn.store(a, c);
+}
+
 template <int P, int T, int NV> PassFn late_entry() {
     if constexpr (WaveStaged<P, T>::value) return pass_kernel_late<P, T, NV>;
     else return nullptr;
diff --git a/reed-solomon-16_amd/csrc/rs16_pass_common.hpp b/reed-solomon-16_amd/csrc/rs16_pass_common.hpp
--- a/reed-solomon-16_amd/csrc/rs16_pass_common.hpp
+++ b/reed-solomon-16_amd/csrc/rs16_pass_common.hpp
@@ -14,6 +14,7 @@
     PassFn late;
     int gather;
     PassFn paired = nullptr;
+    PassFn tower = nullptr;
 };
 struct PassConsts {
     uint32_t nslab, voff32, full_lanes;
@@ -25,6 +26,7 @@
 constexpr int NARROW_VARIANTS = 4;
 PassKernel pass_kernels_enc(int prog, int T, int nv);
 PassKernel pass_kernels_dec(int prog, int T, int nv);
+PassFn pass_kernels_tower(int prog, int T, int nv);
 
 #if defined(__HIPCC__) || defined(__HIP__)
 typedef const __attribute__((address_space(4))) uint32_t* cu32p;
diff --git a/reed-solomon-16_amd/csrc/rs16_pass_launch.hip b/reed-solomon-16_amd/csrc/rs16_pass_launch.hip
--- a/reed-solomon-16_amd/csrc/rs16_pass_launch.hip
+++ b/reed-solomon-16_amd/csrc/rs16_pass_launch.hip
@@ -12,6 +12,7 @@
                 for (int nv = 0; nv < NARROW_VARIANTS; nv++) {
                     const PassKernel e = pass_kernels_enc(prog, T, nv);
                     k[prog][T][nv] = e.fn ? e : pass_kernels_dec(prog, T, nv);
+                    if (k[prog][T][nv].paired) k[prog][T][nv].tower = pass_kernels_tower(prog, T, nv);
                 }
     }
 };
@@ -85,6 +86,16 @@
     return true;
 }
 
+bool tower_rows_sequence(uint32_t chunk_rows, uint64_t S, uint64_t S_user, uint32_t a_count, uint32_t seg_chunk,
+                         uint32_t row_base_in, int diag) {
+    if (diag & DIAG_NO_TOWER_ROWS) return false;
+    if (!paired_rows_sequence(chunk_rows, S, S_user, a_count, seg_chunk, row_base_in, diag)) return false;
+    int L = 0;
+    while (((uint32_t)1 << L) < chunk_rows) L++;
+    const int lo = L / 2, hi = L - lo;
+    return find_kernel(ENC_FIRST, lo, 0).tower && find_kernel(ENC_MID, hi, 0).tower && find_kernel(ENC_LAST, lo, 0).tower;
+}
+
 hipError_t launch_pass(int prog, int T, const PassArgs& args, uint32_t num_tiles, hipStream_t s) {
     if (prog < 0 || prog >= NUM_PROGS || T < 0 || T > 8) return hipErrorInvalidValue;
     if (num_tiles == 0 || args.qrow == 0) return hipSuccess;
@@ -111,9 +122,11 @@
     const size_t lds = (size_t)k.lds;
     PassFn fn = pc.late_rows ? k.late : k.fn;
     if (a.paired) {
-        if (a.paired != paired_sides_of(prog) || !k.paired || !pc.late_rows || !pc.full_lanes)
+        const bool tower = (a.paired & PAIRED_TOWER) != 0;
+        if ((a.paired & ~(uint32_t)PAIRED_TOWER) != paired_sides_of(prog) || !k.paired || !pc.late_rows ||
+            !pc.full_lanes || (tower && !k.tower))
             return hipErrorInvalidValue;
-        fn = k.paired;
+        fn = tower ? k.tower : k.paired;
     }
     if (lds > 65536) {
         hipError_t e = hipFuncSetAttribute((const void*)fn, hipFuncAttributeMaxDynamicSharedMemorySize, (int)lds);
diff --git a/reed-solomon-16_amd/csrc/rs16_pass_tower.hip b/reed-solomon-16_amd/csrc/rs16_pass_tower.hip
--- /dev/null
+++ b/reed-solomon-16_amd/csrc/rs16_pass_tower.hip
@@ -0,0 +1,23 @@
+#include "rs16_pass.hpp"
+
+namespace rs16 {
+
+PassFn pass_kernels_tower(int prog, int T, int nv) {
+    if (prog == ENC_FIRST && T == 7 && nv == 0) return pass_kernel_late_tower<ENC_FIRST, 7, 0>;
+    if (prog == ENC_LAST && T == 7 && nv == 0) return pass_kernel_late_tower<ENC_LAST, 7, 0>;
+    if (prog == ENC_MID && T == 7) {
+        if (nv == 0) return pass_kernel_late_tower<ENC_MID, 7, 0>;
+        if (nv == 1) return pass_kernel_late_tower<ENC_MID, 7, 1>;
+    }
+    if (prog == ENC_MID && T == 8) {
+        switch (nv) {
+            case 0: return pass_kernel_late_tower<ENC_MID, 8, 0>;
+            case 1: return pass_kernel_late_tower<ENC_MID, 8, 1>;
+            case 2: return pass_kernel_late_tower<ENC_MID, 8, 2>;
+            case 3: return pass_kernel_late_tower<ENC_MID, 8, 3>;
+        }
+    }
+    return nullptr;
+}
+
+}
diff --git a/reed-solomon-16_amd/csrc/rs16_tables.cpp b/reed-solomon-16_amd/csrc/rs16_tables.cpp
--- a/reed-solomon-16_amd/csrc/rs16_tables.cpp
+++ b/reed-solomon-16_amd/csrc/rs16_tables.cpp
@@ -17,6 +17,13 @@
 
 inline uint16_t gf_mul(const HostTables& t, uint16_t x, uint32_t log_m) {
     return x == 0 ? 0 : t.exp[add_mod(t.log[x], log_m)];
+}
+
+inline uint16_t tower_conv(const HostTables& t, uint16_t x) {
+    uint16_t r = x;
+    for (int i = 0; i < 8; i++)
+        if ((x >> (8 + i)) & 1) r ^= t.tower_a[i];
+    return r;
 }
 
 void fwht_full(std::vector<uint16_t>& v) {
@@ -112,6 +119,47 @@
             abort();
         }
     }
+
+    for (uint32_t i = 0; i < 8; i++) {
+        const uint16_t a = (uint16_t)((1u << (8 + i)) ^ gf_mul(t, (uint16_t)(1u << i), t.log[1u << 8]));
+        if (a >= 256) {
+            fprintf(stderr, "rs16: basis vector v_%u is not a_i + v_i v_8 with a_i in the subfield\n", 8 + i);
+            abort();
+        }
+        t.tower_a[i] = (uint8_t)a;
+    }
+    for (uint32_t v = 0; v < 8; v++) {
+        t.tower_b[v >> 2] |= (tower_conv(t, (uint16_t)(v << 8)) & 0xFFu) << (8 * (v & 3));
+        t.tower_b[2 + (v >> 2)] |= (tower_conv(t, (uint16_t)(v << 11)) & 0xFFu) << (8 * (v & 3));
+        if (v < 4) t.tower_b[4] |= (tower_conv(t, (uint16_t)(v << 14)) & 0xFFu) << (8 * v);
+    }
+    t.skew_tab_tower.assign((size_t)GF_ORDER * TAB_DWORDS, 0);
+    for (uint32_t i = 0; i < GF_MODULUS; i++) {
+        const uint32_t lm = t.skew_entry[i];
+        if (lm == ZERO_ENTRY) continue;
+        uint32_t* e = &t.skew_tab_tower[(size_t)i * TAB_DWORDS];
+        auto prod = [&](uint32_t x) { return tower_conv(t, gf_mul(t, tower_conv(t, (uint16_t)x), lm)); };
+        for (int g = 0; g < 4; g++)
+            for (uint32_t v = 0; v < 8; v++) {
+                const uint16_t p = prod(v << kOff3[g]);
+                for (int ob = 0; ob < 2; ob++) e[(g * 2 + ob) * 2 + (v >> 2)] |= ((p >> (8 * ob)) & 0xFFu) << (8 * (v & 3));
+            }
+        for (int gg = 0; gg < 2; gg++)
+            for (uint32_t v = 0; v < 4; v++) {
+                const uint16_t p = prod(v << kOff2[gg]);
+                for (int ob = 0; ob < 2; ob++) e[16 + gg * 2 + ob] |= ((p >> (8 * ob)) & 0xFFu) << (8 * v);
+            }
+        if (!twiddle_narrow(i)) continue;
+        const bool cross = (e[2] | e[3] | e[6] | e[7] | e[17] | e[8] | e[9] | e[12] | e[13] | e[18]) != 0;
+        const bool same = e[10] == e[0] && e[11] == e[1] && e[14] == e[4] && e[15] == e[5] && e[19] == e[16];
+        if (cross || !same) {
+            fprintf(stderr, "rs16: tower table of subfield twiddle %u %s\n", i,
+                    cross ? "crosses between the bytes" : "maps the two bytes differently");
+            abort();
+        }
+    }
+    std::copy_n(t.tower_b, 5, &t.skew_tab[TOWER_B_DWORD]);
+    std::copy_n(t.tower_b, 5, &t.skew_tab_tower[TOWER_B_DWORD]);
 
     t.col_img.assign(COL_IMG_DWORDS, 0);
     for (uint32_t L = COL_LMIN; L <= COL_LGEN; L++)
diff --git a/reed-solomon-16_amd/rs16/__init__.py b/reed-solomon-16_amd/rs16/__init__.py
--- a/reed-solomon-16_amd/rs16/__init__.py
+++ b/reed-solomon-16_amd/rs16/__init__.py
@@ -15,7 +15,7 @@
     "supports", "validate", "use_high_rate", "encode_device_batch", "decode_device_batch", "encoder_work_count", "decoder_work_count",
     "RATE_DEFAULT", "RATE_HIGH", "RATE_LOW", "GF_ORDER", "GF_MODULUS", "set_diagnostics",
     "DIAG_FORCE_VOFF64", "DIAG_EVAL_TWO_KERNEL", "DIAG_EVAL_FULL", "DIAG_NO_COLUMN", "DIAG_FORCE_COLUMN",
-    "DIAG_TILE_LAST", "DIAG_NO_TILE_LAST", "DIAG_FD_LDS", "DIAG_COL_RADIX4", "DIAG_NO_IDENTITY", "DIAG_NO_MID_DIRECT", "DIAG_WIDE_TWIDDLES", "DIAG_NO_LATE_ROWS", "DIAG_NO_PAIRED_ROWS", "encode_host", "decode_host",
+    "DIAG_TILE_LAST", "DIAG_NO_TILE_LAST", "DIAG_FD_LDS", "DIAG_COL_RADIX4", "DIAG_NO_IDENTITY", "DIAG_NO_MID_DIRECT", "DIAG_WIDE_TWIDDLES", "DIAG_NO_LATE_ROWS", "DIAG_NO_PAIRED_ROWS", "DIAG_NO_TOWER_ROWS", "encode_host", "decode_host",
     "encode_host_batch", "decode_host_batch", "decode_prepare", "decode_device_prepared",
     "UpdatePlan", "update_recovery_device", "UPDATE_MAX_SHARDS",
     "encode_host_multi", "decode_host_multi", "Comm", "column_slice", "scatter_columns", "gather_columns",
@@ -29,6 +29,7 @@
 DIAG_WIDE_TWIDDLES = 2048
 DIAG_NO_LATE_ROWS = 4096
 DIAG_NO_PAIRED_ROWS = 8192
+DIAG_NO_TOWER_ROWS = 16384
 _diag_default = 0
 
 
diff --git a/reed-solomon-16_amd/rs16/_lib.py b/reed-solomon-16_amd/rs16/_lib.py
--- a/reed-solomon-16_amd/rs16/_lib.py
+++ b/reed-solomon-16_amd/rs16/_lib.py
@@ -35,6 +35,11 @@
                                         C.POINTER(PassConsts)]),
     "rs16_host_pass_consts_many": (_i, [_i, _i, _u32, _sz, _p, _p, _p, _p, _p, _u32, _u32, _u32, _i, _p]),
     "rs16_host_paired_rows": (_i, [_u32, _u64, _u64, _u32, _u32, _u32, _i]),
+    "rs16_host_tower_rows": (_i, [_u32, _u64, _u64, _u32, _u32, _u32, _i]),
+    "rs16_host_tower_basis": (_u32, [_u32]),
+    "rs16_host_tower_conv": (None, [_p, _p, _sz]),
+    "rs16_host_tower_twiddle": (_i, [_u32, C.POINTER(_u32)]),
+    "rs16_host_mul_tower": (None, [_p, _p, _sz, _u32, _i]),
     "rs16_host_update_consts": (_i, [_u32, _u64, _u32, C.POINTER(_u32), C.POINTER(_u32), C.POINTER(_u32),
                                      C.POINTER(_u64)]),
     "rs16_engine_set_profiling": (_i, [_p, _i, _e]),
```

Measured after the change: 1105 GiB/s, median of 6. +2.9%, better.
